# adammoss/nnest

Measured on AMD Instinct MI355X. Metric: live-point evals/sec (flow-transform + loglike) + log-Z error, x_dim=50, higher is better.
Workload: dtype f32

## Files before the change

### nnest_amd/csrc/nnest_solo.hip

```cpp
#include <string.h>
#include <mutex>
#include "mh_common.h"
#include "nnest_internal.h"
#include "solo_loglike.h"
#include "solo_tile.h"

namespace nnest {

#ifdef NNEST_STAMP
#define PSTAMP(v) do { __builtin_amdgcn_sched_barrier(0); v = __builtin_amdgcn_s_memtime(); __builtin_amdgcn_s_waitcnt(0xC07F); __builtin_amdgcn_sched_barrier(0); } while (0)
#define PSTAMP_DRAINED(v) do { __builtin_amdgcn_sched_barrier(0); __builtin_amdgcn_s_waitcnt(0x0070); v = __builtin_amdgcn_s_memtime(); __builtin_amdgcn_s_waitcnt(0xC07F); __builtin_amdgcn_sched_barrier(0); } while (0)
#ifndef NNEST_STAMP_STEPS
#undef STAMP
#define STAMP(v) do { } while (0)
#endif
#else
#define PSTAMP(v) do { } while (0)
#define PSTAMP_DRAINED(v) do { } while (0)
#endif

static constexpr int SOLO_ETAB = 1024;
__device__ double solo_etab_dev[SOLO_ETAB];
__global__ void solo_etab_kernel() {
    const int k = blockIdx.x * blockDim.x + threadIdx.x;
    if (k < SOLO_ETAB) solo_etab_dev[k] = exp(1.0 / (double)(1 + k));
}
hipError_t solo_prepare_device(int device, hipStream_t st) {
    static std::mutex mu;
    static bool done[64];
    std::lock_guard<std::mutex> g(mu);
    if (device < 0 || device >= 64) return hipErrorInvalidDevice;
    if (done[device]) return hipSuccess;
    hipLaunchKernelGGL(solo_etab_kernel, dim3(SOLO_ETAB / 256), dim3(256), 0, st);
    hipError_t e = hipGetLastError();
    if (e == hipSuccess) e = hipStreamSynchronize(st);
    done[device] = e == hipSuccess;
    return e;
}

template <int U>
__global__ void __launch_bounds__(192) solo_image_kernel(const float *__restrict__ packed, float *__restrict__ limg, int D, int net_params) {
    const int lane = threadIdx.x & 63, b = threadIdx.x >> 6;
    SoloNet<U> nb;
    solo_gather<U>(nb, packed + (size_t)(b * 2 + (lane >= 32 ? 1 : 0)) * net_params, D, (b + 1) & 1, b & 1, lane);
    solo4_store<U>(limg, b, nb, lane);
}
hipError_t launch_solo_image(const float *packed, float *limg, const FlowShape &s, hipStream_t st) {
    if (!s.has_solo_image()) return hipErrorInvalidConfiguration;
    switch (s.NT) {
        case 1: hipLaunchKernelGGL(solo_image_kernel<1>, dim3(1), dim3(192), 0, st, packed, limg, s.D, s.net_params); break;
        case 2: hipLaunchKernelGGL(solo_image_kernel<2>, dim3(1), dim3(192), 0, st, packed, limg, s.D, s.net_params); break;
        case 3: hipLaunchKernelGGL(solo_image_kernel<3>, dim3(1), dim3(192), 0, st, packed, limg, s.D, s.net_params); break;
        case 4: hipLaunchKernelGGL(solo_image_kernel<4>, dim3(1), dim3(192), 0, st, packed, limg, s.D, s.net_params); break;
    }
    return hipGetLastError();
}

template <int U, int WPG> constexpr bool solo_lds_weights() { return U >= 3 || WPG > 4; }
template <int U, int WPG> constexpr int solo_reg_blocks() { return !solo_lds_weights<U, WPG>() ? 3 : (WPG == 4 ? 1 : (U <= 2 && WPG == 8 ? 1 : 0)); }

enum { MH_SOLO_LAG_INTERNAL = 8 };
template <int U, bool DBG, int LK, int WPG>
__global__ void __launch_bounds__(64 * (WPG + 2)) mh_kernel_solo(MhArgs a) {
    extern __shared__ __attribute__((aligned(16))) float wlds[];
    __shared__ __attribute__((aligned(16))) float nbuf[2][WPG][16][2 * U];
    __shared__ float ubuf[2][WPG];
    __shared__ __attribute__((aligned(16))) uint32_t rawbuf[4 * WPG * 8 * U];
    __shared__ int acc_lds[2][WPG];
    __shared__ float fsbuf[2];
    __shared__ float fs_exact;
    __shared__ float fs_cand[2];
    __shared__ int vote_sel;
    __shared__ double etab[SOLO_ETAB];
    __shared__ __attribute__((aligned(16))) float x0buf[WPG][16][2 * U];

    const int lane = threadIdx.x & 63, wave = __builtin_amdgcn_readfirstlane(threadIdx.x >> 6);
    const int tile = blockIdx.x;
    const int D = a.s.D, S = a.steps, C = a.C;
    const bool recorded = DBG && a.noise_dz;
    const bool dynamic = (a.flags & NNEST_MH_DYNAMIC_BATCH) != 0;
    const bool use_tab = S + 2 <= SOLO_ETAB;
    const bool exact_all = dynamic && mh_flag_lag(a.flags) == 0;
    const bool direct_votes = (a.flags & NNEST_MH_WINDOW_VOTES_ONLY) == 0;
    const int lag = exact_all ? MH_SOLO_LAG_INTERNAL : mh_flag_lag(a.flags);
    const int warm = dynamic ? min(exact_all ? S : mh_flag_warm(a.flags), S - 1) : 0;
    constexpr bool LDSW = solo_lds_weights<U, WPG>();
    constexpr int RB = solo_reg_blocks<U, WPG>();
    const int ntiles = (C + WPG - 1) / WPG;
    if (tile >= ntiles) {
        if (dynamic && wave == 0) mh_sync_publisher(a.sync, S, exact_all ? S : max(S - lag, warm), ntiles, C, lane, a.sync_err);
        else if (dynamic && (a.flags & (NNEST_MH_SYNC_ZERO_NEXT | NNEST_MH_SYNC_ZERO_PREV))) {
            const size_t W = (size_t)mh_sync_words(S) + 1;
            unsigned long long *other = (a.flags & NNEST_MH_SYNC_ZERO_NEXT) ? a.sync + W : a.sync - W;
            const int nthr = (int)blockDim.x - 64;
            for (size_t i = threadIdx.x - 64; i < W; i += nthr) other[i] = 0ull;
        }
        return;
    }
    unsigned long long p0 = 0, p1 = 0, p2 = 0, p3 = 0, p4 = 0, p5 = 0, p6 = 0, p7 = 0, p8 = 0;
    (void)p0; (void)p1; (void)p2; (void)p3; (void)p4; (void)p5; (void)p6; (void)p7; (void)p8;
    PSTAMP(p0);
    const float *limg = a.img + a.s.solo_image_offset();
    const int j = wave;
    const int pos = lane & 15;
    const bool translate_half = lane >= 32;
    const bool writer_lane = lane < 16;
    const int row = tile * WPG + j;
    const bool ok = row < C;
    SoloNet<U> net[RB > 0 ? RB : 1];
    float z[2][U];
    double logl = 0.0;
    if (wave < WPG) {
        if constexpr (LDSW) {
            if constexpr (RB == 1) solo_image_load<U>(net[0], limg + (size_t)1 * SOLO4_NF * 64, lane);
        } else {
#pragma unroll
            for (int b = 0; b < 3; ++b) solo_image_load<U>(net[b], limg + (size_t)b * SOLO4_NF * 64, lane);
        }
#pragma unroll
        for (int u = 0; u < U; ++u)
#pragma unroll
            for (int c = 0; c < 2; ++c) {
                const int d = 2 * U * pos + 2 * u + c;
                z[c][u] = (ok && d < D) ? a.z[(size_t)row * D + d] : 0.f;
            }
        logl = ok ? a.logl[row] : 0.0;
    }
    if constexpr (LDSW) solo_image_to_lds<64 * (WPG + 2)>(wlds, limg);
    PSTAMP(p1);
    if (dynamic && use_tab)
        for (int k = threadIdx.x; k < S + 2; k += blockDim.x) etab[k] = solo_etab_dev[k];
    PSTAMP(p2);
    __syncthreads();
    PSTAMP(p3);

    if (wave == WPG) {
        const int g = lane & 3, j = min(lane >> 2, WPG - 1);
        const bool gen = lane < 4 * WPG;
        Xoshiro128 rn = xoshiro_seed(a.seed, a.walker_offset + (uint64_t)(tile * WPG + j), (uint32_t)g, NOISE_STREAM_DZ);
        Xoshiro128 ru = xoshiro_seed(a.seed, a.walker_offset + (uint64_t)(tile * WPG + j), 0xffffffffu, NOISE_STREAM_U);
        constexpr int NQ = 8 * WPG * U;
        unsigned long long n0 = 0, n1 = 0, n2 = 0, n_gen = 0, n_all = 0;
        (void)n0; (void)n1; (void)n2; (void)n_gen; (void)n_all;
        auto draw = [&](int k) {
            if (k > S) return;
            STAMP(n0);
            if (!recorded) {
                if (gen) {
#pragma unroll
                    for (int t = 0; t < 2 * U; ++t) {
                        u32x4 r;
                        r.x = xoshiro_next(rn); r.y = xoshiro_next(rn); r.z = xoshiro_next(rn); r.w = xoshiro_next(rn);
                        *reinterpret_cast<u32x4 *>(&rawbuf[lane * 8 * U + 4 * t]) = r;
                    }
                    const float u = xoshiro_uniform(ru);
                    if (g == 0) ubuf[k & 1][j] = u;
                }
                float *nb = &nbuf[k & 1][0][0][0];
#pragma unroll
                for (int i = 0; i < (NQ + 63) / 64; ++i) {
                    const int q = lane + 64 * i;
                    if (NQ % 64 == 0 || q < NQ) {
                        const u32x4 r = *reinterpret_cast<const u32x4 *>(&rawbuf[4 * q]);
                        const int sl = q / (2 * U), qq = q % (2 * U);
                        const int d0 = 32 * (qq >> 1) + 8 * (sl & 3) + 4 * (qq & 1);
                        float o0, o1, o2, o3;
                        box_muller(r.x, r.y, o0, o1);
                        box_muller(r.z, r.w, o2, o3);
                        const f32x4 o = {d0 < D ? o0 : 0.f, d0 + 1 < D ? o1 : 0.f, d0 + 2 < D ? o2 : 0.f, d0 + 3 < D ? o3 : 0.f};
                        *reinterpret_cast<f32x4 *>(nb + (sl >> 2) * 32 * U + d0) = o;
                    }
                }
            }
            if (!dynamic && lane == 0) fsbuf[k & 1] = a.step_size;
            STAMP(n1);
#ifdef NNEST_STAMP
            n_gen += n1 - n0;
#endif
        };
        STAMP(n2);
        draw(0);
        PSTAMP(p4);
        solo_barrier();
        PSTAMP(p5);
        if (S >= 1) {
            draw(1);
            solo_barrier();
            draw(2);
            for (int k = 1; k <= warm; ++k) {
                solo_barrier();
                solo_barrier();
                draw(k + 2);
                solo_barrier();
            }
            for (int k = warm > 0 ? warm + 2 : 2; k <= S; ++k) {
                solo_barrier();
                draw(k + 1);
            }
        }
#ifdef NNEST_STAMP
        { unsigned long long n3 = 0; STAMP(n3); n_all = n3 - n2; }
#endif
#ifdef NNEST_STAMP
        PSTAMP(p8);
        if (a.scale_out && lane == 0 && tile == 0) {
            float *o = a.scale_out;
            o[4] = (float)n_gen; o[5] = (float)n_all;
            o[32] = (float)(p1 - p0); o[33] = (float)(p2 - p1); o[34] = (float)(p3 - p2); o[35] = (float)(p4 - p3); o[36] = (float)(p5 - p4);
            o[37] = (float)(p8 - p5); o[38] = (float)(p8 - p0);
        }
#endif
#ifndef NNEST_STAMP
        if (!dynamic && a.scale_out && lane == 0) {
            const int g0 = (tile * WPG + 15) >> 4;
            if (16 * g0 < (tile + 1) * WPG && 16 * g0 < C) a.scale_out[g0] = a.step_size;
        }
#endif
        return;
    }
    if (wave == WPG + 1) {
        if (!dynamic) return;
        double scale = (double)a.step_size;
        int accept = 0, reject = 0;
        const int last = S - lag;
        const unsigned long long *wbase = a.sync + 2 * mh_sync_counter_words(S) + (size_t)(tile & (MH_SYNC_SHARDS - 1)) * MH_SYNC_STRIDE;
#define SOLO_RELAY_ITERATION(k_, q_)                                                                                        \
        {                                                                                                                   \
            const int k = (k_), want = k - lag;                                                                             \
              \
              \
              \
              \
              \
            asm volatile("s_waitcnt vmcnt(2)" : "+v"(q_) : : "memory");                                                     \
            if (want > warm) {                                                                                              \
                const bool up = mh_window_vote(a.sync, S, want, tile, q_, a.sync_err);                                      \
                if (up) accept += 1; else reject += 1;                                                                      \
                if (accept > reject) scale *= use_tab ? etab[accept] : exp(1.0 / (1 + accept));                             \
                if (accept < reject) scale /= use_tab ? etab[reject] : exp(1.0 / (1 + reject));                             \
            }                                                                                                               \
                   \
             \
            if (lane == 0) {                                                                                                \
                const int *ac = acc_lds[k & 1];                                                                             \
                const bool mine = k - 2 > warm;                                 \
                int acs = 0;                                                                                                \
                _Pragma("unroll") for (int w_ = 0; w_ < WPG; ++w_) acs += ac[w_];                                           \
                mh_sync_post(a.sync, mine ? k - 2 : 0, tile, mine ? acs : 0);                                               \
            }                                                                                                               \
            const int ask = min(max(want + 2, 1), max(last, 1));         \
            const unsigned long long *wp = wbase + (size_t)((ask - 1) >> 5) * MH_SYNC_SHARDS * MH_SYNC_STRIDE;              \
            asm volatile("global_load_dwordx2 %0, %1, off sc1" : "=v"(q_) : "v"(wp) : "memory");                            \
              \
            if (lane == 0) fsbuf[k & 1] = (float)scale;                                                                     \
            solo_barrier();                                                                           \
        }
        unsigned long long qa = 0, qb = 0;
        int k0 = 0;
        if (warm > 0) {
            auto E = [&](int n) { return use_tab ? etab[n] : exp(1.0 / (1 + n)); };
            auto next_scale = [&](int acc, int rej, double sc) {
                if (acc > rej) sc *= E(acc);
                if (acc < rej) sc /= E(rej);
                return sc;
            };
            if (lane == 0) {
                fsbuf[0] = (float)scale;
                fs_cand[0] = (float)next_scale(accept + 1, reject, scale);
                fs_cand[1] = (float)next_scale(accept, reject + 1, scale);
            }
            solo_barrier();
            if (lane == 0) fsbuf[1] = (float)scale;
            solo_barrier();
            for (int k = 1; k <= warm; ++k) {
                solo_barrier();
                if (lane == 0) {
                    const int *ac = acc_lds[k & 1];
                    int acs = 0;
#pragma unroll
                    for (int w_ = 0; w_ < WPG; ++w_) acs += ac[w_];
                    mh_sync_post(a.sync, k, tile, acs);
                    fsbuf[(k + 1) & 1] = (float)scale;
                }
                solo_barrier();
                const bool up = direct_votes ? 2 * mh_sync_total(a.sync, k, ntiles, 0ull, a.sync_err) > C
                                             : mh_window_vote(a.sync, S, k, tile, 0ull, a.sync_err);
                if (up) accept += 1; else reject += 1;
                scale = next_scale(accept, reject, scale);
                if (lane == 0) {
                    vote_sel = up ? 0 : 1;
                    fs_exact = (float)scale;
                    fs_cand[0] = (float)next_scale(accept + 1, reject, scale);
                    fs_cand[1] = (float)next_scale(accept, reject + 1, scale);
                }
                solo_barrier();
            }
            k0 = warm + 2;
        }
        for (int k2 = k0; k2 <= S; k2 += 2) {
            SOLO_RELAY_ITERATION(k2, qa)
            if (k2 + 1 <= S) SOLO_RELAY_ITERATION(k2 + 1, qb)
        }
#undef SOLO_RELAY_ITERATION
        asm volatile("s_waitcnt vmcnt(0)" : "+v"(qa), "+v"(qb) : : "memory");
        if (exact_all) {
            solo_barrier();
            if (lane == 0) {
                const int *ac = acc_lds[S & 1];
                int acs = 0;
#pragma unroll
                for (int w_ = 0; w_ < WPG; ++w_) acs += ac[w_];
                mh_sync_post(a.sync, S, tile, acs);
            }
            const bool up = direct_votes ? 2 * mh_sync_total(a.sync, S, ntiles, 0ull, a.sync_err) > C : mh_window_vote(a.sync, S, S, tile, 0ull, a.sync_err);
            if (up) accept += 1; else reject += 1;
            if (accept > reject) scale *= use_tab ? etab[accept] : exp(1.0 / (1 + accept));
            if (accept < reject) scale /= use_tab ? etab[reject] : exp(1.0 / (1 + reject));
        }
#ifndef NNEST_STAMP
        if (a.scale_out && lane == 0) {
            const int g0 = (tile * WPG + 15) >> 4;
            if (16 * g0 < (tile + 1) * WPG && 16 * g0 < C) a.scale_out[g0] = (float)scale;
        }
#endif
        return;
    }

    const LikeSpec like = a.like;
    const double loglstar = a.loglstar;
    const bool free_mode = (a.flags & NNEST_MH_UNCONSTRAINED) != 0;
    PSTAMP(p4);
    const unsigned sel = translate_half ? 0xffffffffu : 0u;
    const bool h1 = (lane & 16) != 0;
    auto inverse = [&](float (&xs)[2][U]) {
        if constexpr (LDSW) {
            float ld = solo_coupling_inverse4<U>(Solo4Lds{wlds + (size_t)2 * SOLO4_NF * 64, lane}, sel, h1, xs[1], xs[0]);
            if constexpr (RB == 1) ld += solo_coupling_inverse4<U>(Solo4Reg<U>{net[0]}, sel, h1, xs[0], xs[1]);
            else ld += solo_coupling_inverse4<U>(Solo4Lds{wlds + (size_t)1 * SOLO4_NF * 64, lane}, sel, h1, xs[0], xs[1]);
            ld += solo_coupling_inverse4<U>(Solo4Lds{wlds, lane}, sel, h1, xs[1], xs[0]);
            return ld;
        } else {
            float ld;
            solo_coupling_inverse<U, true>(net[2], sel, h1, xs[1], xs[0], ld);
            solo_coupling_inverse<U, false>(net[1], sel, h1, xs[0], xs[1], ld);
            solo_coupling_inverse<U, false>(net[0], sel, h1, xs[1], xs[0], ld);
            return ld;
        }
    };

    float x[2][U];
#pragma unroll
    for (int u = 0; u < U; ++u)
#pragma unroll
        for (int c = 0; c < 2; ++c) x[c][u] = z[c][u];
    float ld = solo_logdet_total(inverse(x));
    int n_acc = 0, n_call = 0;

    auto store_row = [&](float *base, size_t r, const float (&v)[2][U]) {
#pragma unroll
        for (int u = 0; u < U; ++u)
#pragma unroll
            for (int c = 0; c < 2; ++c) {
                const int d = 2 * U * pos + 2 * u + c;
                if (d < D) base[r * D + d] = v[c][u];
            }
    };
    if (writer_lane && a.x) {
#pragma unroll
        for (int u = 0; u < U; ++u)
#pragma unroll
            for (int c = 0; c < 2; ++c) x0buf[j][pos][2 * u + c] = x[c][u];
    }
    if (DBG && writer_lane && ok) {
        if (a.hist_x) store_row(a.hist_x, (size_t)row * (S + 1), x);
        if (a.hist_logl && pos == 0) a.hist_logl[(size_t)row * (S + 1)] = logl;
    }

    float nz[2 * U], u_next = 0.f, fs_next = a.step_size;
    int kbuf = 0;
    auto fetch_noise = [&]() {
        solo_barrier();
        if (!recorded) {
#pragma unroll
            for (int k = 0; k < 2 * U; ++k) nz[k] = nbuf[kbuf & 1][j][pos][k];
            u_next = ubuf[kbuf & 1][j];
        }
        fs_next = fsbuf[kbuf & 1];
        ++kbuf;
    };
    PSTAMP(p5);
    fetch_noise();
    PSTAMP(p6);

    unsigned long long st0 = 0, st1 = 0, st2 = 0, st3 = 0, a_prop = 0, a_inv = 0, a_post = 0, a_tot = 0;
    (void)st0; (void)st1; (void)st2; (void)st3; (void)a_prop; (void)a_inv; (void)a_post; (void)a_tot;
    struct Prop { float zp[2][U], xp[2][U]; float ldp; double lp; bool pre, acc; };
    auto propose = [&](int it, float fs, float (&zp)[2][U], float &u) {
        if (recorded) {
#pragma unroll
            for (int uu = 0; uu < U; ++uu)
#pragma unroll
                for (int c = 0; c < 2; ++c) {
                    const int d = 2 * U * pos + 2 * uu + c;
                    const float dz = (ok && d < D) ? a.noise_dz[((size_t)(it - 1) * C + row) * D + d] : 0.f;
                    zp[c][uu] = __builtin_fmaf(dz, fs, z[c][uu]);
                }
            u = ok ? a.noise_u[(size_t)(it - 1) * C + row] : 1.f;
        } else {
#pragma unroll
            for (int uu = 0; uu < U; ++uu) {
                zp[0][uu] = __builtin_fmaf(nz[2 * uu], fs, z[0][uu]);
                zp[1][uu] = __builtin_fmaf(nz[2 * uu + 1], fs, z[1][uu]);
            }
            u = u_next;
        }
    };
    auto finish = [&](Prop &r, float u) {
#pragma unroll
        for (int c = 0; c < 2; ++c)
#pragma unroll
            for (int uu = 0; uu < U; ++uu) r.xp[c][uu] = r.zp[c][uu];
        STAMP(st1);
        constexpr bool RIDE = LK == NNEST_LIKE_ROSENBROCK;
        r.ldp = RIDE ? inverse(r.xp) : solo_logdet_total(inverse(r.xp));
        STAMP(st2);
        if constexpr (RIDE) r.lp = solo_loglike<U, LK>(like, D, lane, r.xp, &r.ldp);
        int okl = 1;
#pragma unroll
        for (int c = 0; c < 2; ++c)
#pragma unroll
            for (int uu = 0; uu < U; ++uu) okl &= !(r.xp[c][uu] < -1.f || r.xp[c][uu] > 1.f);
        const bool inb = __ballot(okl != 0) == ~0ull;
        float log_ratio = inb ? (r.ldp - ld) : -INFINITY;
        float ratio = fminf(__expf(log_ratio), 1.0f);
        if (log_ratio != log_ratio) ratio = log_ratio;
        r.pre = ok && (u < ratio);
        if constexpr (!RIDE) r.lp = solo_loglike<U, LK>(like, D, lane, r.xp);
        r.acc = r.pre && (r.lp > loglstar);
        if (free_mode) {
            const double lr = inb ? (double)(r.ldp - ld) + (r.lp - logl) : -INFINITY;
            const double rt = fmin(exp(lr), 1.0);
            r.acc = ok && ((double)u < rt);
        }
    };
    auto apply = [&](int it, const Prop &r) {
        n_call += (free_mode ? ok : r.pre) ? 1 : 0;
        n_acc += r.acc ? 1 : 0;
#pragma unroll
        for (int c = 0; c < 2; ++c)
#pragma unroll
            for (int uu = 0; uu < U; ++uu) {
                z[c][uu] = r.acc ? r.zp[c][uu] : z[c][uu];
                x[c][uu] = r.acc ? r.xp[c][uu] : x[c][uu];
            }
        ld = r.acc ? r.ldp : ld;
        logl = r.acc ? r.lp : logl;
        if (dynamic && lane == 0) acc_lds[it & 1][j] = r.acc ? 1 : 0;
        if (DBG && writer_lane && ok) {
            if (a.hist_x) store_row(a.hist_x, (size_t)row * (S + 1) + it, x);
            if (a.hist_logl && pos == 0) a.hist_logl[(size_t)row * (S + 1) + it] = logl;
        }
    };
    Prop cur;
    bool have = false;
    for (int it = 1; it <= S; ++it) {
        STAMP(st0);
        if (!have) {
            float u;
            propose(it, fs_next, cur.zp, u);
            fetch_noise();
            finish(cur, u);
        }
        apply(it, cur);
        have = false;
        if (it <= warm) {
            solo_barrier();
            const float f0 = fs_cand[0], f1 = fs_cand[1];
            Prop c1;
            float u;
            propose(it + 1, f0, cur.zp, u);
            propose(it + 1, f1, c1.zp, u);
            fetch_noise();
            finish(cur, u);
            finish(c1, u);
            solo_barrier();
            if (vote_sel != 0) cur = c1;
            have = true;
            fs_next = fs_exact;
        }
        STAMP(st3);
#ifdef NNEST_STAMP
        a_prop += st1 - st0; a_inv += st2 - st1; a_post += st3 - st2; a_tot += st3 - st0;
#endif
    }
    if (exact_all) solo_barrier();
    PSTAMP(p7);
#ifdef NNEST_STAMP
    if (a.scale_out && lane == 0 && tile == 0) {
        float *o = a.scale_out;
        if (j == 0) { o[0] = (float)a_tot; o[1] = (float)a_prop; o[2] = (float)a_inv; o[3] = (float)a_post; }
        if (j < 4) { o[8 + 2 * j] = (float)a_inv; o[9 + 2 * j] = (float)a_post; }
    }
#endif
    bool all_moved = n_acc > 0;
    if (a.x) {
        bool mine = true;
        if (writer_lane) {
#pragma unroll
            for (int u = 0; u < U; ++u)
#pragma unroll
                for (int c = 0; c < 2; ++c) {
                    const int d = 2 * U * pos + 2 * u + c;
                    const float x0 = x0buf[j][pos][2 * u + c];
                    mine = mine && (d >= D || x[c][u] != x0);
                }
        }
        all_moved = (__ballot(mine) & 0xffffull) == 0xffffull;
    }
    if (writer_lane && ok) {
        store_row(a.z, (size_t)row, z);
        if (a.x) store_row(a.x, (size_t)row, x);
        if (pos == 0) {
            a.logl[row] = logl;
            if (a.n_accept) a.n_accept[row] = n_acc | (all_moved ? NNEST_MH_ALL_MOVED : 0);
            if (a.n_call) a.n_call[row] = n_call;
        }
    }
#ifdef NNEST_STAMP
    PSTAMP_DRAINED(p8);
    if (a.scale_out && lane == 0 && tile == 0 && j == 0) {
        float *o = a.scale_out;
        o[16] = (float)(p1 - p0); o[17] = (float)(p2 - p1); o[18] = (float)(p3 - p2); o[19] = (float)(p4 - p3); o[20] = (float)(p5 - p4);
        o[21] = (float)(p6 - p5); o[22] = (float)(p7 - p6); o[23] = (float)(p8 - p7); o[24] = (float)(p8 - p0);
    }
#endif
}

template <int U>
static __device__ __forceinline__ void slice_normals(uint64_t seed, uint64_t walker, uint32_t step, int pos, int D, float (&e)[2][U]) {
    const int d0 = 2 * U * pos;
    f32x4 q[(2 * U + 3) / 4 + 1];
    const int q0 = d0 >> 2;
#pragma unroll
    for (int k = 0; k < (2 * U + 3) / 4 + 1; ++k) q[k] = noise_normal4(seed, walker, step, (uint32_t)(q0 + k), NOISE_STREAM_DZ);
#pragma unroll
    for (int u = 0; u < U; ++u)
#pragma unroll
        for (int c = 0; c < 2; ++c) {
            const int d = d0 + 2 * u + c, k = (d >> 2) - q0, r = d & 3;
            float v = 0.f;
#pragma unroll
            for (int kk = 0; kk < (2 * U + 3) / 4 + 1; ++kk)
                if (kk == k) v = r == 0 ? q[kk].x : (r == 1 ? q[kk].y : (r == 2 ? q[kk].z : q[kk].w));
            e[c][u] = d < D ? v : 0.f;
        }
}

template <int U, int LK>
__global__ void __launch_bounds__(256) slice_kernel_solo(SliceArgs a, FlowShape s, const float *limg) {
    extern __shared__ __attribute__((aligned(16))) float wlds[];
    __shared__ __attribute__((aligned(16))) float x0buf[4][16][2 * U];
    const int lane = threadIdx.x & 63, wave = __builtin_amdgcn_readfirstlane(threadIdx.x >> 6);
    const int D = s.D, S = a.steps, C = a.C;
    constexpr bool LDSW = solo_lds_weights<U, 4>();
    if constexpr (LDSW) {
        solo_image_to_lds<256>(wlds, limg);
        __syncthreads();
    }
    const int pos = lane & 15;
    const bool translate_half = lane >= 32, writer_lane = lane < 16;
    const int row = blockIdx.x * 4 + wave;
    const bool ok = row < C;
    if (!ok) return;
    const LikeSpec like = a.like;
    const double loglstar = a.loglstar;
    SoloNet<U> net[LDSW ? 1 : 3];
    if constexpr (!LDSW) {
#pragma unroll
        for (int b = 0; b < 3; ++b) solo_image_load<U>(net[b], limg + (size_t)b * SOLO4_NF * 64, lane);
    }
    const unsigned sel = translate_half ? 0xffffffffu : 0u;
    const bool h1 = (lane & 16) != 0;
    auto inverse = [&](float (&xs)[2][U]) {
        if constexpr (LDSW) {
            float ld = solo_coupling_inverse4<U>(Solo4Lds{wlds + (size_t)2 * SOLO4_NF * 64, lane}, sel, h1, xs[1], xs[0]);
            ld += solo_coupling_inverse4<U>(Solo4Lds{wlds + (size_t)1 * SOLO4_NF * 64, lane}, sel, h1, xs[0], xs[1]);
            ld += solo_coupling_inverse4<U>(Solo4Lds{wlds, lane}, sel, h1, xs[1], xs[0]);
            return ld;
        } else {
            float ld;
            solo_coupling_inverse<U, true>(net[2], sel, h1, xs[1], xs[0], ld);
            solo_coupling_inverse<U, false>(net[1], sel, h1, xs[0], xs[1], ld);
            solo_coupling_inverse<U, false>(net[0], sel, h1, xs[1], xs[0], ld);
            return ld;
        }
    };
    auto store_row = [&](float *base, size_t r, const float (&v)[2][U]) {
#pragma unroll
        for (int u = 0; u < U; ++u)
#pragma unroll
            for (int c = 0; c < 2; ++c) {
                const int d = 2 * U * pos + 2 * u + c;
                if (d < D) base[r * D + d] = v[c][u];
            }
    };
    float z[2][U], x[2][U];
#pragma unroll
    for (int u = 0; u < U; ++u)
#pragma unroll
        for (int c = 0; c < 2; ++c) {
            const int d = 2 * U * pos + 2 * u + c;
            z[c][u] = d < D ? a.z[(size_t)row * D + d] : 0.f;
            x[c][u] = z[c][u];
        }
    float ld = solo_logdet_total(inverse(x));
    double logl = a.logl[row];
    if (writer_lane && a.x) {
#pragma unroll
        for (int u = 0; u < U; ++u)
#pragma unroll
            for (int c = 0; c < 2; ++c) x0buf[wave][pos][2 * u + c] = x[c][u];
    }
    if (writer_lane && a.hist_x) store_row(a.hist_x, (size_t)row * (S + 1), x);
    const uint64_t walker = a.walker_offset + (uint64_t)row;
    int n_call = 0, n_move = 0, n_eval = 0;
    float zc[2][U], xc[2][U], ldc = 0.f;
    double lc = 0.0;
    for (int it = 1; it <= S; ++it) {
        float e[2][U];
        if (a.noise_dz) {
#pragma unroll
            for (int u = 0; u < U; ++u)
#pragma unroll
                for (int c = 0; c < 2; ++c) {
                    const int d = 2 * U * pos + 2 * u + c;
                    e[c][u] = d < D ? a.noise_dz[((size_t)(it - 1) * C + row) * D + d] : 0.f;
                }
        } else {
            slice_normals<U>(a.seed, walker, (uint32_t)it, pos, D, e);
        }
        const float u0 = noise_uniform(a.seed, walker, 64u * (uint32_t)it + 0u), u1 = noise_uniform(a.seed, walker, 64u * (uint32_t)it + 1u);
        const float logy = ld + __logf(u1);
        auto inside = [&](float t) -> bool {
            const float tw = t * a.width;
#pragma unroll
            for (int u = 0; u < U; ++u)
#pragma unroll
                for (int c = 0; c < 2; ++c) { zc[c][u] = __builtin_fmaf(e[c][u], tw, z[c][u]); xc[c][u] = zc[c][u]; }
            ldc = solo_logdet_total(inverse(xc));
            int okl = 1;
#pragma unroll
            for (int c = 0; c < 2; ++c)
#pragma unroll
                for (int u = 0; u < U; ++u) okl &= !(xc[c][u] < -1.f || xc[c][u] > 1.f);
            const bool inb = __ballot(okl != 0) == ~0ull;
            const bool pre = inb && (ldc > logy);
            lc = solo_loglike<U, LK>(like, D, lane, xc);
            n_eval += 1;
            n_call += pre ? 1 : 0;
            return pre && (lc > loglstar);
        };
        float tl = -u0, tr = 1.0f - u0;
        if (a.max_out > 0) {
            const int B = 2 * a.max_out;
            int n = 0;
            while (n <= B && inside(tl)) { tl -= 1.0f; n += 1; }
            while (n <= B && inside(tr)) { tr += 1.0f; n += 1; }
            if (n > B) {
                tl = -u0;
                tr = 1.0f - u0;
                const int nl = slice_stepout_left(a.seed, walker, (uint32_t)it, a.max_out);
                for (int j = 0; j < nl; ++j) { if (!inside(tl)) break; tl -= 1.0f; }
                for (int j = 0; j < B - nl; ++j) { if (!inside(tr)) break; tr += 1.0f; }
            }
        }
        bool moved = false;
        for (int k = 0; k < a.max_shrink; ++k) {
            const float uk = noise_uniform(a.seed, walker, 64u * (uint32_t)it + 2u + (uint32_t)k);
            const float t = __builtin_fmaf(tr - tl, uk, tl);
            if (inside(t)) { moved = true; break; }
            if (t < 0.f) tl = t; else tr = t;
        }
        if (moved) {
#pragma unroll
            for (int c = 0; c < 2; ++c)
#pragma unroll
                for (int u = 0; u < U; ++u) { z[c][u] = zc[c][u]; x[c][u] = xc[c][u]; }
            ld = ldc; logl = lc; n_move += 1;
        }
        if (writer_lane && a.hist_x) store_row(a.hist_x, (size_t)row * (S + 1) + it, x);
    }
    bool all_moved = n_move > 0;
    if (a.x) {
        bool mine = true;
        if (writer_lane) {
#pragma unroll
            for (int u = 0; u < U; ++u)
#pragma unroll
                for (int c = 0; c < 2; ++c) {
                    const int d = 2 * U * pos + 2 * u + c;
                    const float x0 = x0buf[wave][pos][2 * u + c];
                    mine = mine && (d >= D || x[c][u] != x0);
                }
        }
        all_moved = (__ballot(mine) & 0xffffull) == 0xffffull;
    }
    if (writer_lane) {
        store_row(a.z, (size_t)row, z);
        if (a.x) store_row(a.x, (size_t)row, x);
        if (pos == 0) {
            a.logl[row] = logl;
            if (a.n_call) a.n_call[row] = n_call;
            if (a.n_move) a.n_move[row] = n_move | (all_moved ? NNEST_MH_ALL_MOVED : 0);
            if (a.n_eval) a.n_eval[row] = n_eval;
        }
    }
}

__global__ void slice_fill_noise_kernel(float *__restrict__ dz, int steps, int C, int D, uint64_t seed, uint64_t walker_offset) {
    const long nq = (long)steps * C * ((D + 3) / 4);
    for (long i = (long)blockIdx.x * blockDim.x + threadIdx.x; i < nq; i += (long)gridDim.x * blockDim.x) {
        const int Q = (D + 3) / 4, q = (int)(i % Q), c = (int)((i / Q) % C), it = (int)(i / ((long)Q * C)) + 1;
        const f32x4 n = noise_normal4(seed, walker_offset + (uint64_t)c, (uint32_t)it, (uint32_t)q, NOISE_STREAM_DZ);
        float *o = dz + ((size_t)(it - 1) * C + c) * D + 4 * q;
        if (4 * q + 0 < D) o[0] = n.x;
        if (4 * q + 1 < D) o[1] = n.y;
        if (4 * q + 2 < D) o[2] = n.z;
        if (4 * q + 3 < D) o[3] = n.w;
    }
}

template <int U, int LK>
static hipError_t launch_slice_k(const FlowShape &s, const float *limg, const SliceArgs &a, hipStream_t st) {
    const size_t lds = solo_lds_weights<U, 4>() ? (size_t)3 * SOLO4_NF * 64 * sizeof(float) : 0;
    hipError_t e = hipFuncSetAttribute(reinterpret_cast<const void *>(slice_kernel_solo<U, LK>), hipFuncAttributeMaxDynamicSharedMemorySize, (int)lds);
    if (e != hipSuccess) return e;
    hipLaunchKernelGGL((slice_kernel_solo<U, LK>), dim3((a.C + 3) / 4), dim3(256), lds, st, a, s, limg);
    return hipGetLastError();
}

bool slice_form_eligible(const FlowShape &s) {
    return s.kind == FLOW_KIND_NVP && s.H == 16 && s.B == 3 && s.L == 1 && s.scale_mode == 0 && s.NT >= 1 && s.NT <= 4;
}

hipError_t launch_slice_solo(const FlowShape &s, const float *limg, const SliceArgs &a, hipStream_t st) {
    if (a.C <= 0) return hipSuccess;
    if (!slice_form_eligible(s)) return hipErrorInvalidConfiguration;
    const bool rosen = a.like.id == NNEST_LIKE_ROSENBROCK;
    switch (s.NT) {
        case 1: return rosen ? launch_slice_k<1, NNEST_LIKE_ROSENBROCK>(s, limg, a, st) : launch_slice_k<1, -1>(s, limg, a, st);
        case 2: return rosen ? launch_slice_k<2, NNEST_LIKE_ROSENBROCK>(s, limg, a, st) : launch_slice_k<2, -1>(s, limg, a, st);
        case 3: return rosen ? launch_slice_k<3, NNEST_LIKE_ROSENBROCK>(s, limg, a, st) : launch_slice_k<3, -1>(s, limg, a, st);
        case 4: return rosen ? launch_slice_k<4, NNEST_LIKE_ROSENBROCK>(s, limg, a, st) : launch_slice_k<4, -1>(s, limg, a, st);
    }
    return hipErrorInvalidConfiguration;
}

hipError_t launch_slice_fill_noise(float *dz, int steps, int C, int D, uint64_t seed, uint64_t walker_offset, hipStream_t st) {
    hipLaunchKernelGGL(slice_fill_noise_kernel, dim3(256), dim3(256), 0, st, dz, steps, C, D, seed, walker_offset);
    return hipGetLastError();
}

int solo_walkers_per_group(int C, int num_cu) {
    static const int pinned = [] { const char *e = getenv("NNEST_SOLO_WPG"); return e ? atoi(e) : 0; }();
    for (int wpg = 4; wpg <= 12; wpg += 4) {
        if (pinned && wpg != pinned) continue;
        if ((C + wpg - 1) / wpg + 1 <= num_cu) return wpg;
    }
    return 0;
}

bool solo_form_eligible(const MhArgs &a, int num_cu) {
    const FlowShape &s = a.s;
    if (s.H != 16 || s.B != 3 || s.L != 1 || s.scale_mode != 0 || s.NT < 1 || s.NT > 4) return false;
    if (a.flags & NNEST_MH_DYNAMIC_STEP) return false;
    if ((a.flags & NNEST_MH_DYNAMIC_BATCH) && (mh_flag_lag(a.flags) == 1 || mh_flag_lag(a.flags) == 2)) return false;
    const int wpg = solo_walkers_per_group(a.C, num_cu);
    if (wpg != 4 && (a.noise_dz || a.hist_x || a.hist_logl)) return false;
    return wpg != 0;
}

template <int U, bool DBG, int LK, int WPG>
static hipError_t launch_solo_k(const MhArgs &a, hipStream_t st) {
    const int batch = (a.flags & NNEST_MH_DYNAMIC_BATCH) ? 1 : 0;
    const int grid = (a.C + WPG - 1) / WPG + batch;
    const size_t lds = solo_lds_weights<U, WPG>() ? (size_t)3 * SOLO4_NF * 64 * sizeof(float) : 0;
    hipError_t e = hipFuncSetAttribute(reinterpret_cast<const void *>(mh_kernel_solo<U, DBG, LK, WPG>),
                                       hipFuncAttributeMaxDynamicSharedMemorySize, (int)lds);
    if (e != hipSuccess) return e;
    hipLaunchKernelGGL((mh_kernel_solo<U, DBG, LK, WPG>), dim3(grid), dim3(64 * (WPG + 2)), lds, st, a);
    return hipGetLastError();
}
template <int U, bool DBG, int LK>
static hipError_t launch_solo_w(const MhArgs &a, int wpg, hipStream_t st) {
    if (wpg == 4) return launch_solo_k<U, DBG, LK, 4>(a, st);
    if constexpr (!DBG) {
        if (wpg == 8) return launch_solo_k<U, DBG, LK, 8>(a, st);
        if (wpg == 12) return launch_solo_k<U, DBG, LK, 12>(a, st);
    }
    return hipErrorInvalidConfiguration;
}

hipError_t launch_mh_solo(const MhArgs &a_in, int num_cu, hipStream_t st) {
    MhArgs a = a_in;
    static const bool window_votes = [] { const char *e = getenv("NNEST_SOLO_VOTE"); return e && !strcmp(e, "window"); }();
    if (window_votes) a.flags |= NNEST_MH_WINDOW_VOTES_ONLY;
    const bool dbg = a.noise_dz || a.hist_x || a.hist_logl;
    const int wpg = solo_walkers_per_group(a.C, num_cu);
    if (!dbg && a.like.id == NNEST_LIKE_ROSENBROCK) {
        if (a.s.NT == 1) return launch_solo_w<1, false, NNEST_LIKE_ROSENBROCK>(a, wpg, st);
        if (a.s.NT == 2) return launch_solo_w<2, false, NNEST_LIKE_ROSENBROCK>(a, wpg, st);
        if (a.s.NT == 3) return launch_solo_w<3, false, NNEST_LIKE_ROSENBROCK>(a, wpg, st);
        if (a.s.NT == 4) return launch_solo_w<4, false, NNEST_LIKE_ROSENBROCK>(a, wpg, st);
    }
    switch (a.s.NT) {
        case 1: return dbg ? launch_solo_w<1, true, -1>(a, wpg, st) : launch_solo_w<1, false, -1>(a, wpg, st);
        case 2: return dbg ? launch_solo_w<2, true, -1>(a, wpg, st) : launch_solo_w<2, false, -1>(a, wpg, st);
        case 3: return dbg ? launch_solo_w<3, true, -1>(a, wpg, st) : launch_solo_w<3, false, -1>(a, wpg, st);
        case 4: return dbg ? launch_solo_w<4, true, -1>(a, wpg, st) : launch_solo_w<4, false, -1>(a, wpg, st);
    }
    return hipErrorInvalidConfiguration;
}

}
```

Before: 941.8 million.

## Restructure solo MH loop into warm and unrolled straight phases, defer x inverse

Splits the MH step loop into a warm-up phase and a straight phase unrolled by two, so the LDS double-buffer parity is a compile-time constant instead of a running counter. Proposal registers are pinned across the noise-fetch barrier to steer scheduling. When neither DBG nor LDS weights are in use, x is no longer selected at every step; it is rebuilt once at the end by running the inverse flow on z. The intent is to cut per-step register moves and selects, at the cost of one extra flow inverse per chain and extra code size.

```diff
diff --git a/nnest_amd/csrc/nnest_solo.hip b/nnest_amd/csrc/nnest_solo.hip
--- a/nnest_amd/csrc/nnest_solo.hip
+++ b/nnest_amd/csrc/nnest_solo.hip
@@ -3,6 +3,7 @@
 #include "mh_common.h"
 #include "nnest_internal.h"
 #include "solo_loglike.h"
+#include "solo_schedule.h"
 #include "solo_tile.h"
 
 namespace nnest {
@@ -58,6 +59,14 @@
 
 template <int U, int WPG> constexpr bool solo_lds_weights() { return U >= 3 || WPG > 4; }
 template <int U, int WPG> constexpr int solo_reg_blocks() { return !solo_lds_weights<U, WPG>() ? 3 : (WPG == 4 ? 1 : (U <= 2 && WPG == 8 ? 1 : 0)); }
+
+template <int U>
+static __device__ __forceinline__ void solo_pin(float (&v)[2][U]) {
+#pragma unroll
+    for (int c = 0; c < 2; ++c)
+#pragma unroll
+        for (int u = 0; u < U; ++u) asm volatile("" : "+v"(v[c][u]));
+}
 
 enum { MH_SOLO_LAG_INTERNAL = 8 };
 template <int U, bool DBG, int LK, int WPG>
@@ -83,7 +92,7 @@
     const bool exact_all = dynamic && mh_flag_lag(a.flags) == 0;
     const bool direct_votes = (a.flags & NNEST_MH_WINDOW_VOTES_ONLY) == 0;
     const int lag = exact_all ? MH_SOLO_LAG_INTERNAL : mh_flag_lag(a.flags);
-    const int warm = dynamic ? min(exact_all ? S : mh_flag_warm(a.flags), S - 1) : 0;
+    const int warm = solo_warm_steps(S, mh_flag_warm(a.flags), dynamic, exact_all);
     constexpr bool LDSW = solo_lds_weights<U, WPG>();
     constexpr int RB = solo_reg_blocks<U, WPG>();
     const int ntiles = (C + WPG - 1) / WPG;
@@ -193,7 +202,7 @@
                 draw(k + 2);
                 solo_barrier();
             }
-            for (int k = warm > 0 ? warm + 2 : 2; k <= S; ++k) {
+            for (int k = solo_first_lagged_fetch(warm); k <= S; ++k) {
                 solo_barrier();
                 draw(k + 1);
             }
@@ -256,7 +265,7 @@
             solo_barrier();                                                                           \
         }
         unsigned long long qa = 0, qb = 0;
-        int k0 = 0;
+        const int k0 = solo_relay_first_iteration(warm);
         if (warm > 0) {
             auto E = [&](int n) { return use_tab ? etab[n] : exp(1.0 / (1 + n)); };
             auto next_scale = [&](int acc, int rej, double sc) {
@@ -295,7 +304,6 @@
                 }
                 solo_barrier();
             }
-            k0 = warm + 2;
         }
         for (int k2 = k0; k2 <= S; k2 += 2) {
             SOLO_RELAY_ITERATION(k2, qa)
@@ -348,6 +356,7 @@
         }
     };
 
+    constexpr bool X_LATE = !DBG && !LDSW;
     float x[2][U];
 #pragma unroll
     for (int u = 0; u < U; ++u)
@@ -377,19 +386,18 @@
     }
 
     float nz[2 * U], u_next = 0.f, fs_next = a.step_size;
-    int kbuf = 0;
-    auto fetch_noise = [&]() {
+    auto fetch_noise = [&](int par, auto &...zp) {
         solo_barrier();
+        (solo_pin(zp), ...);
         if (!recorded) {
 #pragma unroll
-            for (int k = 0; k < 2 * U; ++k) nz[k] = nbuf[kbuf & 1][j][pos][k];
-            u_next = ubuf[kbuf & 1][j];
-        }
-        fs_next = fsbuf[kbuf & 1];
-        ++kbuf;
+            for (int k = 0; k < 2 * U; ++k) nz[k] = nbuf[par][j][pos][k];
+            u_next = ubuf[par][j];
+        }
+        fs_next = fsbuf[par];
     };
     PSTAMP(p5);
-    fetch_noise();
+    fetch_noise(0);
     PSTAMP(p6);
 
     unsigned long long st0 = 0, st1 = 0, st2 = 0, st3 = 0, a_prop = 0, a_inv = 0, a_post = 0, a_tot = 0;
@@ -443,7 +451,7 @@
             r.acc = ok && ((double)u < rt);
         }
     };
-    auto apply = [&](int it, const Prop &r) {
+    auto apply = [&](int it, int par, const Prop &r) {
         n_call += (free_mode ? ok : r.pre) ? 1 : 0;
         n_acc += r.acc ? 1 : 0;
 #pragma unroll
@@ -451,47 +459,67 @@
 #pragma unroll
             for (int uu = 0; uu < U; ++uu) {
                 z[c][uu] = r.acc ? r.zp[c][uu] : z[c][uu];
-                x[c][uu] = r.acc ? r.xp[c][uu] : x[c][uu];
+                if constexpr (!X_LATE) x[c][uu] = r.acc ? r.xp[c][uu] : x[c][uu];
             }
         ld = r.acc ? r.ldp : ld;
         logl = r.acc ? r.lp : logl;
-        if (dynamic && lane == 0) acc_lds[it & 1][j] = r.acc ? 1 : 0;
+        if (dynamic && lane == 0) acc_lds[par][j] = r.acc ? 1 : 0;
         if (DBG && writer_lane && ok) {
             if (a.hist_x) store_row(a.hist_x, (size_t)row * (S + 1) + it, x);
             if (a.hist_logl && pos == 0) a.hist_logl[(size_t)row * (S + 1) + it] = logl;
         }
     };
-    Prop cur;
-    bool have = false;
-    for (int it = 1; it <= S; ++it) {
-        STAMP(st0);
-        if (!have) {
+    if (warm > 0) {
+        Prop cur;
+        {
             float u;
-            propose(it, fs_next, cur.zp, u);
-            fetch_noise();
+            propose(1, fs_next, cur.zp, u);
+            fetch_noise(1, cur.zp);
             finish(cur, u);
         }
-        apply(it, cur);
-        have = false;
-        if (it <= warm) {
+        for (int it = 1; it <= warm; ++it) {
+            STAMP(st0);
+            apply(it, it & 1, cur);
             solo_barrier();
             const float f0 = fs_cand[0], f1 = fs_cand[1];
             Prop c1;
             float u;
             propose(it + 1, f0, cur.zp, u);
             propose(it + 1, f1, c1.zp, u);
-            fetch_noise();
+            fetch_noise((it + 1) & 1, cur.zp, c1.zp);
             finish(cur, u);
             finish(c1, u);
             solo_barrier();
             if (vote_sel != 0) cur = c1;
-            have = true;
             fs_next = fs_exact;
-        }
+            STAMP(st3);
+#ifdef NNEST_STAMP
+            a_prop += st1 - st0; a_inv += st2 - st1; a_post += st3 - st2; a_tot += st3 - st0;
+#endif
+        }
+        apply(warm + 1, (warm + 1) & 1, cur);
+    }
+    auto straight_step = [&](int it, int par) {
+        STAMP(st0);
+        Prop r;
+        float u;
+        propose(it, fs_next, r.zp, u);
+        fetch_noise(par, r.zp);
+        finish(r, u);
+        apply(it, par, r);
         STAMP(st3);
 #ifdef NNEST_STAMP
         a_prop += st1 - st0; a_inv += st2 - st1; a_post += st3 - st2; a_tot += st3 - st0;
 #endif
+    };
+    {
+        int it = solo_first_straight_step(warm);
+        if (it <= S && (it & 1)) { straight_step(it, 1); ++it; }
+        for (; it < S; it += 2) {
+            straight_step(it, 0);
+            straight_step(it + 1, 1);
+        }
+        if (it <= S) straight_step(it, 0);
     }
     if (exact_all) solo_barrier();
     PSTAMP(p7);
@@ -504,6 +532,13 @@
 #endif
     bool all_moved = n_acc > 0;
     if (a.x) {
+        if constexpr (X_LATE) {
+#pragma unroll
+            for (int u = 0; u < U; ++u)
+#pragma unroll
+                for (int c = 0; c < 2; ++c) x[c][u] = z[c][u];
+            (void)inverse(x);
+        }
         bool mine = true;
         if (writer_lane) {
 #pragma unroll
diff --git a/nnest_amd/csrc/solo_schedule.h b/nnest_amd/csrc/solo_schedule.h
--- /dev/null
+++ b/nnest_amd/csrc/solo_schedule.h
@@ -0,0 +1,45 @@
+#pragma once
+
+#if defined(__HIPCC__) || defined(__CUDACC__)
+#define SOLO_SCHED_FN __host__ __device__ constexpr
+#else
+#define SOLO_SCHED_FN constexpr
+#endif
+
+namespace nnest {
+
+SOLO_SCHED_FN int solo_warm_steps(int S, int flag_warm, bool dynamic, bool exact_all) {
+    return dynamic ? ((exact_all ? S : flag_warm) < S - 1 ? (exact_all ? S : flag_warm) : S - 1) : 0;
+}
+SOLO_SCHED_FN int solo_first_straight_step(int warm) { return warm > 0 ? warm + 2 : 1; }
+SOLO_SCHED_FN int solo_first_lagged_fetch(int warm) { return warm > 0 ? warm + 2 : 2; }
+SOLO_SCHED_FN int solo_lagged_fetches(int S, int warm) { return S >= solo_first_lagged_fetch(warm) ? S - solo_first_lagged_fetch(warm) + 1 : 0; }
+SOLO_SCHED_FN int solo_relay_first_iteration(int warm) { return warm > 0 ? warm + 2 : 0; }
+
+SOLO_SCHED_FN int solo_net_barriers(int S, int warm, bool dynamic, bool exact_all) {
+    int n = 1;
+    if (warm > 0) n += 1 + 3 * warm;
+    const int first = solo_first_straight_step(warm);
+    n += S >= first ? S - first + 1 : 0;
+    return n + (exact_all ? 1 : 0);
+}
+SOLO_SCHED_FN int solo_noise_barriers(int S, int warm, bool dynamic, bool exact_all) {
+    int n = 1;
+    if (S >= 1) n += 1 + 3 * warm + solo_lagged_fetches(S, warm);
+    return n;
+}
+SOLO_SCHED_FN int solo_relay_barriers(int S, int warm, bool dynamic, bool exact_all) {
+    if (!dynamic) return 0;
+    int n = warm > 0 ? 2 + 3 * warm : 0;
+    const int k0 = solo_relay_first_iteration(warm);
+    n += S >= k0 ? S - k0 + 1 : 0;
+    return n + (exact_all ? 1 : 0);
+}
+SOLO_SCHED_FN int solo_noise_barriers_due(int S, int warm, bool dynamic, bool exact_all) {
+    return solo_net_barriers(S, warm, dynamic, exact_all) - (exact_all ? 1 : 0);
+}
+SOLO_SCHED_FN int solo_relay_barriers_due(int S, int warm, bool dynamic, bool exact_all) {
+    return dynamic ? solo_net_barriers(S, warm, dynamic, exact_all) : 0;
+}
+
+}
diff --git a/profiles/r09/k4_solo_loop.s b/profiles/r09/k4_solo_loop.s
--- /dev/null
+++ b/profiles/r09/k4_solo_loop.s
@@ -0,0 +1,812 @@
+	v_mov_b32_e32 v193, s70
+	ds_write_b32 v193, v185 offset:16
+	s_or_b64 exec, exec, s[12:13]
+	v_and_b32_e32 v186, 0xffff, v186
+	v_and_b32_e32 v147, 0xffff, v147
+	s_add_i32 s19, s19, 2
+	v_add3_u32 v168, v168, v186, v147
+	v_add3_u32 v169, v169, v187, v185
+	v_cndmask_b32_e64 v29, v29, v190, s[14:15]
+	v_cndmask_b32_e64 v93, v93, v191, s[14:15]
+	v_cndmask_b32_e64 v143, v143, v189, s[14:15]
+	v_cndmask_b32_e64 v145, v145, v167, s[14:15]
+	v_cndmask_b32_e64 v144, v144, v166, s[14:15]
+	v_cndmask_b32_e64 v177, v177, v192, s[14:15]
+	s_cmp_lt_i32 s19, s29
+	v_cndmask_b32_e64 v89, v89, v188, s[14:15]
+	s_cbranch_scc0 1220
+	s_waitcnt lgkmcnt(0)
+	v_fma_f32 v189, v138, v171, v29
+	v_fma_f32 v188, v139, v171, v143
+	v_fma_f32 v190, v140, v171, v93
+	v_fma_f32 v171, v141, v171, v89
+	s_waitcnt lgkmcnt(0)
+	s_barrier
+	v_mov_b32_e32 v198, v146
+	v_mov_b32_e32 v147, v188
+	v_mov_b32_e32 v166, v171
+	v_bfi_b32 v187, v173, v190, v189
+	v_mov_b32_dpp v147, v188 row_ror:8 row_mask:0xa bank_mask:0xf
+	v_mov_b32_dpp v166, v171 row_ror:8 row_mask:0xa bank_mask:0xf
+	v_fma_f32 v167, v147, v94, v90
+	v_mul_f32_e32 v186, v166, v102
+	v_fmac_f32_dpp v186, v166, v103 row_ror:1 row_mask:0xf bank_mask:0xf
+	v_fmac_f32_dpp v167, v147, v95 row_ror:1 row_mask:0xf bank_mask:0xf
+	v_fmac_f32_dpp v186, v166, v104 row_ror:2 row_mask:0xf bank_mask:0xf
+	v_fmac_f32_dpp v167, v147, v96 row_ror:2 row_mask:0xf bank_mask:0xf
+	v_fmac_f32_dpp v186, v166, v105 row_ror:3 row_mask:0xf bank_mask:0xf
+	v_fmac_f32_dpp v167, v147, v97 row_ror:3 row_mask:0xf bank_mask:0xf
+	v_fmac_f32_dpp v186, v166, v106 row_ror:4 row_mask:0xf bank_mask:0xf
+	v_fmac_f32_dpp v167, v147, v98 row_ror:4 row_mask:0xf bank_mask:0xf
+	v_fmac_f32_dpp v186, v166, v107 row_ror:5 row_mask:0xf bank_mask:0xf
+	v_fmac_f32_dpp v167, v147, v99 row_ror:5 row_mask:0xf bank_mask:0xf
+	v_fmac_f32_dpp v186, v166, v108 row_ror:6 row_mask:0xf bank_mask:0xf
+	v_fmac_f32_dpp v167, v147, v100 row_ror:6 row_mask:0xf bank_mask:0xf
+	v_fmac_f32_dpp v186, v166, v109 row_ror:7 row_mask:0xf bank_mask:0xf
+	v_fmac_f32_dpp v167, v147, v101 row_ror:7 row_mask:0xf bank_mask:0xf
+	v_add_f32_e32 v166, v167, v186
+	v_mov_b32_dpp v147, v186 row_ror:8 row_mask:0xf bank_mask:0xf
+	v_add_f32_dpp v147, v167, v147 row_ror:8 row_mask:0xf bank_mask:0xf
+	s_nop 1
+	v_permlane16_swap_b32_e32 v166, v147
+	v_add_f32_e32 v167, v166, v147
+	v_exp_f32_e32 v147, v167
+	v_max_f32_e32 v166, 0, v167
+	v_add_f32_e32 v147, 1.0, v147
+	v_rcp_f32_e32 v147, v147
+	s_nop 0
+	v_fma_f32 v147, v147, -2.0, 1.0
+	v_bfi_b32 v167, v142, v166, v147
+	v_fma_f32 v147, v167, v110, v91
+	s_nop 0
+	v_mul_f32_dpp v166, v167, v111 row_ror:1 row_mask:0xf bank_mask:0xf
+	v_fmac_f32_dpp v147, v167, v112 row_ror:2 row_mask:0xf bank_mask:0xf
+	v_fmac_f32_dpp v166, v167, v113 row_ror:3 row_mask:0xf bank_mask:0xf
+	v_fmac_f32_dpp v147, v167, v114 row_ror:4 row_mask:0xf bank_mask:0xf
+	v_fmac_f32_dpp v166, v167, v115 row_ror:5 row_mask:0xf bank_mask:0xf
+	v_fmac_f32_dpp v147, v167, v116 row_ror:6 row_mask:0xf bank_mask:0xf
+	v_fmac_f32_dpp v166, v167, v117 row_ror:7 row_mask:0xf bank_mask:0xf
+	v_add_f32_e32 v167, v147, v166
+	v_add_f32_e32 v186, v147, v166
+	s_nop 1
+	v_permlane16_swap_b32_e32 v167, v186
+	v_add_f32_e32 v167, v167, v186
+	v_exp_f32_e32 v147, v167
+	v_max_f32_e32 v166, 0, v167
+	v_add_f32_e32 v147, 1.0, v147
+	v_rcp_f32_e32 v147, v147
+	s_nop 0
+	v_fma_f32 v147, v147, -2.0, 1.0
+	v_bfi_b32 v167, v142, v166, v147
+	v_fma_f32 v147, v167, v118, v92
+	v_mov_b32_e32 v166, 0
+	v_fmac_f32_dpp v166, v167, v122 row_ror:8 row_mask:0xf bank_mask:0xf
+	v_fmac_f32_dpp v147, v167, v119 row_ror:1 row_mask:0xf bank_mask:0xf
+	v_fmac_f32_dpp v166, v167, v123 row_ror:9 row_mask:0xf bank_mask:0xf
+	v_fmac_f32_dpp v147, v167, v120 row_ror:2 row_mask:0xf bank_mask:0xf
+	v_fmac_f32_dpp v166, v167, v124 row_ror:10 row_mask:0xf bank_mask:0xf
+	v_fmac_f32_dpp v147, v167, v121 row_ror:3 row_mask:0xf bank_mask:0xf
+	v_fmac_f32_dpp v166, v167, v125 row_ror:11 row_mask:0xf bank_mask:0xf
+	v_fmac_f32_dpp v147, v167, v126 row_ror:4 row_mask:0xf bank_mask:0xf
+	v_fmac_f32_dpp v166, v167, v130 row_ror:12 row_mask:0xf bank_mask:0xf
+	v_fmac_f32_dpp v147, v167, v127 row_ror:5 row_mask:0xf bank_mask:0xf
+	v_fmac_f32_dpp v166, v167, v131 row_ror:13 row_mask:0xf bank_mask:0xf
+	v_fmac_f32_dpp v147, v167, v128 row_ror:6 row_mask:0xf bank_mask:0xf
+	v_fmac_f32_dpp v166, v167, v132 row_ror:14 row_mask:0xf bank_mask:0xf
+	v_fmac_f32_dpp v147, v167, v129 row_ror:7 row_mask:0xf bank_mask:0xf
+	v_fmac_f32_dpp v166, v167, v133 row_ror:15 row_mask:0xf bank_mask:0xf
+	v_add_f32_e32 v167, v147, v166
+	v_add_f32_e32 v186, v147, v166
+	s_nop 1
+	v_permlane32_swap_b32_e32 v167, v186
+	v_mul_f32_e32 v147, 0xbfb8aa3b, v167
+	v_exp_f32_e32 v147, v147
+	v_sub_f32_e32 v166, v187, v186
+	v_mul_f32_e32 v193, v166, v147
+	v_mul_f32_e32 v194, v166, v147
+	v_mul_f32_e32 v191, -1.0, v167
+	s_nop 0
+	v_permlane16_swap_b32_e32 v193, v194
+	ds_read_b128 v[138:141], v176
+	ds_read_b32 v185, v178
+	ds_read_b32 v192, v179 offset:12352
+	v_mov_b32_e32 v147, v193
+	v_mov_b32_e32 v167, v194
+	v_bfi_b32 v195, v173, v171, v188
+	v_mov_b32_dpp v147, v193 row_ror:8 row_mask:0xa bank_mask:0xf
+	v_mov_b32_dpp v167, v194 row_ror:8 row_mask:0xa bank_mask:0xf
+	v_fma_f32 v186, v147, v50, v86
+	v_mul_f32_e32 v187, v167, v34
+	v_fmac_f32_dpp v187, v167, v35 row_ror:1 row_mask:0xf bank_mask:0xf
+	v_fmac_f32_dpp v186, v147, v51 row_ror:1 row_mask:0xf bank_mask:0xf
+	v_fmac_f32_dpp v187, v167, v36 row_ror:2 row_mask:0xf bank_mask:0xf
+	v_fmac_f32_dpp v186, v147, v52 row_ror:2 row_mask:0xf bank_mask:0xf
+	v_fmac_f32_dpp v187, v167, v37 row_ror:3 row_mask:0xf bank_mask:0xf
+	v_fmac_f32_dpp v186, v147, v53 row_ror:3 row_mask:0xf bank_mask:0xf
+	v_fmac_f32_dpp v187, v167, v58 row_ror:4 row_mask:0xf bank_mask:0xf
+	v_fmac_f32_dpp v186, v147, v54 row_ror:4 row_mask:0xf bank_mask:0xf
+	v_fmac_f32_dpp v187, v167, v59 row_ror:5 row_mask:0xf bank_mask:0xf
+	v_fmac_f32_dpp v186, v147, v55 row_ror:5 row_mask:0xf bank_mask:0xf
+	v_fmac_f32_dpp v187, v167, v60 row_ror:6 row_mask:0xf bank_mask:0xf
+	v_fmac_f32_dpp v186, v147, v56 row_ror:6 row_mask:0xf bank_mask:0xf
+	v_fmac_f32_dpp v187, v167, v61 row_ror:7 row_mask:0xf bank_mask:0xf
+	v_fmac_f32_dpp v186, v147, v57 row_ror:7 row_mask:0xf bank_mask:0xf
+	v_add_f32_e32 v167, v186, v187
+	v_mov_b32_dpp v147, v187 row_ror:8 row_mask:0xf bank_mask:0xf
+	v_add_f32_dpp v147, v186, v147 row_ror:8 row_mask:0xf bank_mask:0xf
+	s_nop 1
+	v_permlane16_swap_b32_e32 v167, v147
+	v_add_f32_e32 v186, v167, v147
+	v_exp_f32_e32 v147, v186
+	v_max_f32_e32 v167, 0, v186
+	v_add_f32_e32 v147, 1.0, v147
+	v_rcp_f32_e32 v147, v147
+	s_nop 0
+	v_fma_f32 v147, v147, -2.0, 1.0
+	v_bfi_b32 v186, v142, v167, v147
+	v_fma_f32 v147, v186, v62, v87
+	s_nop 0
+	v_mul_f32_dpp v167, v186, v63 row_ror:1 row_mask:0xf bank_mask:0xf
+	v_fmac_f32_dpp v147, v186, v64 row_ror:2 row_mask:0xf bank_mask:0xf
+	v_fmac_f32_dpp v167, v186, v65 row_ror:3 row_mask:0xf bank_mask:0xf
+	v_fmac_f32_dpp v147, v186, v66 row_ror:4 row_mask:0xf bank_mask:0xf
+	v_fmac_f32_dpp v167, v186, v67 row_ror:5 row_mask:0xf bank_mask:0xf
+	v_fmac_f32_dpp v147, v186, v68 row_ror:6 row_mask:0xf bank_mask:0xf
+	v_fmac_f32_dpp v167, v186, v69 row_ror:7 row_mask:0xf bank_mask:0xf
+	v_add_f32_e32 v186, v147, v167
+	v_add_f32_e32 v187, v147, v167
+	s_nop 1
+	v_permlane16_swap_b32_e32 v186, v187
+	v_add_f32_e32 v186, v186, v187
+	v_exp_f32_e32 v147, v186
+	v_max_f32_e32 v167, 0, v186
+	v_add_f32_e32 v147, 1.0, v147
+	v_rcp_f32_e32 v147, v147
+	s_nop 0
+	v_fma_f32 v147, v147, -2.0, 1.0
+	v_bfi_b32 v186, v142, v167, v147
+	v_fma_f32 v147, v186, v70, v88
+	v_mov_b32_e32 v167, 0
+	v_fmac_f32_dpp v167, v186, v78 row_ror:8 row_mask:0xf bank_mask:0xf
+	v_fmac_f32_dpp v147, v186, v71 row_ror:1 row_mask:0xf bank_mask:0xf
+	v_fmac_f32_dpp v167, v186, v79 row_ror:9 row_mask:0xf bank_mask:0xf
+	v_fmac_f32_dpp v147, v186, v72 row_ror:2 row_mask:0xf bank_mask:0xf
+	v_fmac_f32_dpp v167, v186, v80 row_ror:10 row_mask:0xf bank_mask:0xf
+	v_fmac_f32_dpp v147, v186, v73 row_ror:3 row_mask:0xf bank_mask:0xf
+	v_fmac_f32_dpp v167, v186, v81 row_ror:11 row_mask:0xf bank_mask:0xf
+	v_fmac_f32_dpp v147, v186, v74 row_ror:4 row_mask:0xf bank_mask:0xf
+	v_fmac_f32_dpp v167, v186, v82 row_ror:12 row_mask:0xf bank_mask:0xf
+	v_fmac_f32_dpp v147, v186, v75 row_ror:5 row_mask:0xf bank_mask:0xf
+	v_fmac_f32_dpp v167, v186, v83 row_ror:13 row_mask:0xf bank_mask:0xf
+	v_fmac_f32_dpp v147, v186, v76 row_ror:6 row_mask:0xf bank_mask:0xf
+	v_fmac_f32_dpp v167, v186, v84 row_ror:14 row_mask:0xf bank_mask:0xf
+	v_fmac_f32_dpp v147, v186, v77 row_ror:7 row_mask:0xf bank_mask:0xf
+	v_fmac_f32_dpp v167, v186, v85 row_ror:15 row_mask:0xf bank_mask:0xf
+	v_add_f32_e32 v186, v147, v167
+	v_add_f32_e32 v187, v147, v167
+	s_nop 1
+	v_permlane32_swap_b32_e32 v186, v187
+	v_mul_f32_e32 v147, 0xbfb8aa3b, v186
+	v_exp_f32_e32 v147, v147
+	v_sub_f32_e32 v167, v195, v187
+	v_mul_f32_e32 v166, v167, v147
+	v_mul_f32_e32 v202, v167, v147
+	v_sub_f32_e32 v191, v191, v186
+	s_nop 0
+	v_permlane16_swap_b32_e32 v166, v202
+	s_nop 0
+	v_mov_b32_e32 v147, v166
+	v_mov_b32_e32 v187, v202
+	v_bfi_b32 v197, v173, v194, v193
+	v_mov_b32_dpp v147, v166 row_ror:8 row_mask:0xa bank_mask:0xf
+	v_mov_b32_dpp v187, v202 row_ror:8 row_mask:0xa bank_mask:0xf
+	v_fma_f32 v195, v147, v30, v26
+	v_mul_f32_e32 v196, v187, v42
+	v_fmac_f32_dpp v196, v187, v43 row_ror:1 row_mask:0xf bank_mask:0xf
+	v_fmac_f32_dpp v195, v147, v31 row_ror:1 row_mask:0xf bank_mask:0xf
+	v_fmac_f32_dpp v196, v187, v44 row_ror:2 row_mask:0xf bank_mask:0xf
+	v_fmac_f32_dpp v195, v147, v32 row_ror:2 row_mask:0xf bank_mask:0xf
+	v_fmac_f32_dpp v196, v187, v45 row_ror:3 row_mask:0xf bank_mask:0xf
+	v_fmac_f32_dpp v195, v147, v33 row_ror:3 row_mask:0xf bank_mask:0xf
+	v_fmac_f32_dpp v196, v187, v46 row_ror:4 row_mask:0xf bank_mask:0xf
+	v_fmac_f32_dpp v195, v147, v38 row_ror:4 row_mask:0xf bank_mask:0xf
+	v_fmac_f32_dpp v196, v187, v47 row_ror:5 row_mask:0xf bank_mask:0xf
+	v_fmac_f32_dpp v195, v147, v39 row_ror:5 row_mask:0xf bank_mask:0xf
+	v_fmac_f32_dpp v196, v187, v48 row_ror:6 row_mask:0xf bank_mask:0xf
+	v_fmac_f32_dpp v195, v147, v40 row_ror:6 row_mask:0xf bank_mask:0xf
+	v_fmac_f32_dpp v196, v187, v49 row_ror:7 row_mask:0xf bank_mask:0xf
+	v_fmac_f32_dpp v195, v147, v41 row_ror:7 row_mask:0xf bank_mask:0xf
+	v_add_f32_e32 v187, v195, v196
+	v_mov_b32_dpp v147, v196 row_ror:8 row_mask:0xf bank_mask:0xf
+	v_add_f32_dpp v147, v195, v147 row_ror:8 row_mask:0xf bank_mask:0xf
+	s_nop 1
+	v_permlane16_swap_b32_e32 v187, v147
+	v_add_f32_e32 v195, v187, v147
+	v_exp_f32_e32 v147, v195
+	v_max_f32_e32 v187, 0, v195
+	v_add_f32_e32 v147, 1.0, v147
+	v_rcp_f32_e32 v147, v147
+	s_nop 0
+	v_fma_f32 v147, v147, -2.0, 1.0
+	v_bfi_b32 v195, v142, v187, v147
+	v_fma_f32 v147, v195, v6, v27
+	s_nop 0
+	v_mul_f32_dpp v187, v195, v7 row_ror:1 row_mask:0xf bank_mask:0xf
+	v_fmac_f32_dpp v147, v195, v8 row_ror:2 row_mask:0xf bank_mask:0xf
+	v_fmac_f32_dpp v187, v195, v9 row_ror:3 row_mask:0xf bank_mask:0xf
+	v_fmac_f32_dpp v147, v195, v14 row_ror:4 row_mask:0xf bank_mask:0xf
+	v_fmac_f32_dpp v187, v195, v15 row_ror:5 row_mask:0xf bank_mask:0xf
+	v_fmac_f32_dpp v147, v195, v16 row_ror:6 row_mask:0xf bank_mask:0xf
+	v_fmac_f32_dpp v187, v195, v17 row_ror:7 row_mask:0xf bank_mask:0xf
+	v_add_f32_e32 v195, v147, v187
+	v_add_f32_e32 v196, v147, v187
+	s_nop 1
+	v_permlane16_swap_b32_e32 v195, v196
+	v_add_f32_e32 v195, v195, v196
+	v_exp_f32_e32 v147, v195
+	v_max_f32_e32 v187, 0, v195
+	v_add_f32_e32 v147, 1.0, v147
+	v_rcp_f32_e32 v147, v147
+	s_nop 0
+	v_fma_f32 v147, v147, -2.0, 1.0
+	v_bfi_b32 v195, v142, v187, v147
+	v_fma_f32 v147, v195, v2, v28
+	v_mov_b32_e32 v187, 0
+	v_fmac_f32_dpp v187, v195, v18 row_ror:8 row_mask:0xf bank_mask:0xf
+	v_fmac_f32_dpp v147, v195, v3 row_ror:1 row_mask:0xf bank_mask:0xf
+	v_fmac_f32_dpp v187, v195, v19 row_ror:9 row_mask:0xf bank_mask:0xf
+	v_fmac_f32_dpp v147, v195, v4 row_ror:2 row_mask:0xf bank_mask:0xf
+	v_fmac_f32_dpp v187, v195, v20 row_ror:10 row_mask:0xf bank_mask:0xf
+	v_fmac_f32_dpp v147, v195, v5 row_ror:3 row_mask:0xf bank_mask:0xf
+	v_fmac_f32_dpp v187, v195, v21 row_ror:11 row_mask:0xf bank_mask:0xf
+	v_fmac_f32_dpp v147, v195, v10 row_ror:4 row_mask:0xf bank_mask:0xf
+	v_fmac_f32_dpp v187, v195, v22 row_ror:12 row_mask:0xf bank_mask:0xf
+	v_fmac_f32_dpp v147, v195, v11 row_ror:5 row_mask:0xf bank_mask:0xf
+	v_fmac_f32_dpp v187, v195, v23 row_ror:13 row_mask:0xf bank_mask:0xf
+	v_fmac_f32_dpp v147, v195, v12 row_ror:6 row_mask:0xf bank_mask:0xf
+	v_fmac_f32_dpp v187, v195, v24 row_ror:14 row_mask:0xf bank_mask:0xf
+	v_fmac_f32_dpp v147, v195, v13 row_ror:7 row_mask:0xf bank_mask:0xf
+	v_fmac_f32_dpp v187, v195, v25 row_ror:15 row_mask:0xf bank_mask:0xf
+	v_add_f32_e32 v195, v147, v187
+	v_add_f32_e32 v196, v147, v187
+	s_nop 1
+	v_permlane32_swap_b32_e32 v195, v196
+	v_mul_f32_e32 v147, 0xbfb8aa3b, v195
+	v_exp_f32_e32 v147, v147
+	v_sub_f32_e32 v187, v197, v196
+	v_mul_f32_e32 v167, v187, v147
+	v_mul_f32_e32 v186, v187, v147
+	v_sub_f32_e32 v191, v191, v195
+	s_nop 0
+	v_permlane16_swap_b32_e32 v167, v186
+	s_nop 0
+	v_pk_mul_f32 v[194:195], s[52:53], v[166:167]
+	v_mov_b32_e32 v187, v166
+	v_pk_mul_f32 v[196:197], s[52:53], v[186:187]
+	v_pk_mul_f32 v[200:201], v[194:195], v[194:195] neg_lo:[0,1] neg_hi:[0,1]
+	v_mov_b32_dpp v199, v195 row_ror:15 row_mask:0xf bank_mask:0xf bound_ctrl:1
+	v_pk_add_f32 v[200:201], v[196:197], v[200:201]
+	v_pk_add_f32 v[194:195], v[194:195], 1.0 op_sel_hi:[1,0] neg_lo:[1,0] neg_hi:[1,0]
+	v_pk_mul_f32 v[200:201], v[200:201], v[200:201]
+	v_pk_mul_f32 v[194:195], v[194:195], v[194:195]
+	v_pk_mul_f32 v[200:201], v[200:201], s[18:19] op_sel_hi:[1,0]
+	s_nop 0
+	v_pk_add_f32 v[194:195], v[194:195], v[200:201]
+	s_nop 0
+	v_cndmask_b32_e64 v147, 0, v195, s[2:3]
+	v_cndmask_b32_e64 v187, 0, v194, s[4:5]
+	v_pk_mul_f32 v[194:195], v[196:197], v[196:197]
+	v_add_f32_e32 v187, v187, v147
+	v_mul_f32_e32 v147, s52, v202
+	v_mov_b32_e32 v197, v194
+	v_pk_add_f32 v[194:195], v[146:147], v[196:197] neg_lo:[0,1] neg_hi:[0,1]
+	s_nop 0
+	v_pk_mul_f32 v[194:195], v[194:195], v[194:195]
+	s_nop 0
+	v_mul_f32_e32 v193, 0x42c80000, v195
+	v_add_f32_e32 v193, v194, v193
+	v_mul_f32_e32 v195, v147, v147
+	v_mov_b32_e32 v194, v147
+	v_pk_add_f32 v[194:195], v[198:199], v[194:195] neg_lo:[0,1] neg_hi:[0,1]
+	v_cndmask_b32_e64 v193, 0, v193, s[6:7]
+	v_pk_mul_f32 v[194:195], v[194:195], v[194:195]
+	v_add_f32_e32 v187, v193, v187
+	v_mul_f32_e32 v147, 0x42c80000, v195
+	v_add_f32_e32 v147, v194, v147
+	v_cndmask_b32_e64 v147, 0, v147, s[8:9]
+	v_add_f32_e32 v147, v147, v187
+	s_nop 1
+	v_add_f32_dpp v191, v191, v191 row_ror:8 row_mask:0xf bank_mask:0xf bound_ctrl:1
+	v_add_f32_dpp v147, v147, v147 row_ror:8 row_mask:0xf bank_mask:0xf bound_ctrl:1
+	s_nop 0
+	v_add_f32_dpp v191, v191, v191 row_ror:4 row_mask:0xf bank_mask:0xf bound_ctrl:1
+	v_add_f32_dpp v147, v147, v147 row_ror:4 row_mask:0xf bank_mask:0xf bound_ctrl:1
+	s_nop 0
+	v_add_f32_dpp v191, v191, v191 row_ror:2 row_mask:0xf bank_mask:0xf bound_ctrl:1
+	v_add_f32_dpp v147, v147, v147 row_ror:2 row_mask:0xf bank_mask:0xf bound_ctrl:1
+	s_nop 0
+	v_add_f32_dpp v187, v191, v191 row_ror:1 row_mask:0xf bank_mask:0xf bound_ctrl:1
+	v_add_f32_dpp v191, v191, v191 row_ror:1 row_mask:0xf bank_mask:0xf bound_ctrl:1
+	v_add_f32_dpp v147, v147, v147 row_ror:1 row_mask:0xf bank_mask:0xf bound_ctrl:1
+	s_nop 0
+	v_permlane16_swap_b32_e32 v191, v187
+	v_add_f32_e32 v191, v191, v187
+	s_nop 0
+	v_cvt_f64_f32_e32 v[194:195], v147
+	v_max3_f32 v147, |v202|, |v166|, |v186|
+	v_max_f32_e64 v166, |v167|, |v167|
+	v_max_f32_e32 v147, v147, v166
+	v_cmp_nlt_f32_e32 vcc, 1.0, v147
+	s_cmp_eq_u64 vcc, -1
+	v_sub_f32_e32 v147, v191, v177
+	s_cselect_b64 s[12:13], -1, 0
+	v_cndmask_b32_e64 v186, v182, v147, s[12:13]
+	v_mul_f32_e32 v166, 0x3fb8aa3b, v186
+	v_exp_f32_e32 v187, v166
+	v_cmp_le_f64_e64 vcc, |v[194:195]|, s[54:55]
+	v_min_f32_e32 v187, 1.0, v187
+	s_nop 0
+	v_cndmask_b32_e64 v167, v180, -v195, vcc
+	v_cndmask_b32_e32 v166, v181, v194, vcc
+	v_cmp_u_f32_e32 vcc, v186, v186
+	v_cmp_lt_f64_e64 s[14:15], s[26:27], v[166:167]
+	s_nop 0
+	v_cndmask_b32_e32 v186, v187, v186, vcc
+	v_cmp_lt_f32_e32 vcc, v170, v186
+	s_and_b64 s[68:69], s[50:51], vcc
+	s_and_b64 vcc, exec, s[10:11]
+	s_and_b64 s[14:15], s[68:69], s[14:15]
+	s_cbranch_vccnz 62
+	v_cvt_f64_f32_e32 v[186:187], v147
+	v_add_f64 v[194:195], v[166:167], -v[144:145]
+	v_add_f64 v[186:187], v[194:195], v[186:187]
+	v_cndmask_b32_e64 v187, v183, v187, s[12:13]
+	v_cndmask_b32_e64 v186, 0, v186, s[12:13]
+	v_mul_f64 v[194:195], v[186:187], s[56:57]
+	v_rndne_f64_e32 v[194:195], v[194:195]
+	v_fma_f64 v[196:197], s[58:59], v[194:195], v[186:187]
+	v_fmac_f64_e32 v[196:197], s[60:61], v[194:195]
+	v_mov_b64_e32 v[198:199], v[148:149]
+	v_fmac_f64_e32 v[198:199], s[62:63], v[196:197]
+	v_mov_b64_e32 v[200:201], v[150:151]
+	v_fmac_f64_e32 v[200:201], v[196:197], v[198:199]
+	v_mov_b64_e32 v[198:199], v[152:153]
+	v_fmac_f64_e32 v[198:199], v[196:197], v[200:201]
+	v_mov_b64_e32 v[200:201], v[154:155]
+	v_fmac_f64_e32 v[200:201], v[196:197], v[198:199]
+	v_mov_b64_e32 v[198:199], v[156:157]
+	v_fmac_f64_e32 v[198:199], v[196:197], v[200:201]
+	v_mov_b64_e32 v[200:201], v[158:159]
+	v_fmac_f64_e32 v[200:201], v[196:197], v[198:199]
+	v_mov_b64_e32 v[198:199], v[160:161]
+	v_fmac_f64_e32 v[198:199], v[196:197], v[200:201]
+	v_mov_b64_e32 v[200:201], v[162:163]
+	v_fmac_f64_e32 v[200:201], v[196:197], v[198:199]
+	v_mov_b64_e32 v[198:199], v[164:165]
+	v_fmac_f64_e32 v[198:199], v[196:197], v[200:201]
+	v_fma_f64 v[198:199], v[196:197], v[198:199], 1.0
+	v_fma_f64 v[196:197], v[196:197], v[198:199], 1.0
+	v_cvt_i32_f64_e32 v147, v[194:195]
+	v_ldexp_f64 v[194:195], v[196:197], v147
+	v_min_f64 v[194:195], v[194:195], 1.0
+	v_cmp_nlt_f64_e32 vcc, s[64:65], v[186:187]
+	v_cmp_ngt_f64_e64 s[12:13], s[66:67], v[186:187]
+	s_andn2_b64 s[14:15], s[14:15], exec
+	v_cndmask_b32_e32 v147, v184, v195, vcc
+	s_and_b64 vcc, s[12:13], vcc
+	v_cndmask_b32_e64 v187, 0, v147, s[12:13]
+	v_cndmask_b32_e32 v186, 0, v194, vcc
+	v_cvt_f64_f32_e32 v[194:195], v170
+	v_cmp_gt_f64_e32 vcc, v[186:187], v[194:195]
+	s_and_b64 s[12:13], s[50:51], vcc
+	s_and_b64 s[12:13], s[12:13], exec
+	s_or_b64 s[14:15], s[14:15], s[12:13]
+	v_mov_b32_e32 v186, v175
+	v_cndmask_b32_e64 v187, 0, 1, s[14:15]
+	s_and_saveexec_b64 s[12:13], s[16:17]
+	s_cbranch_execnz 6
+	s_branch 8
+	v_cndmask_b32_e64 v186, 0, 1, s[68:69]
+	v_cndmask_b32_e64 v187, 0, 1, s[14:15]
+	s_and_saveexec_b64 s[12:13], s[16:17]
+	v_mov_b32_e32 v147, s70
+	ds_write_b32 v147, v187
+	s_or_b64 exec, exec, s[12:13]
+	v_cndmask_b32_e64 v29, v29, v189, s[14:15]
+	v_cndmask_b32_e64 v93, v93, v190, s[14:15]
+	v_cndmask_b32_e64 v143, v143, v188, s[14:15]
+	v_cndmask_b32_e64 v89, v89, v171, s[14:15]
+	v_cndmask_b32_e64 v177, v177, v191, s[14:15]
+	s_waitcnt lgkmcnt(0)
+	v_fma_f32 v190, v138, v192, v29
+	v_fma_f32 v189, v139, v192, v143
+	v_fma_f32 v191, v140, v192, v93
+	v_fma_f32 v188, v141, v192, v89
+	v_mov_b32_e32 v147, s81
+	v_cndmask_b32_e64 v145, v145, v167, s[14:15]
+	v_cndmask_b32_e64 v144, v144, v166, s[14:15]
+	s_waitcnt lgkmcnt(0)
+	s_barrier
+	ds_read_b128 v[138:141], v176 offset:1024
+	ds_read_b32 v170, v147 offset:16
+	ds_read_b32 v171, v179 offset:12356
+	v_mov_b32_e32 v147, v189
+	v_mov_b32_e32 v166, v188
+	v_bfi_b32 v194, v173, v191, v190
+	v_mov_b32_dpp v147, v189 row_ror:8 row_mask:0xa bank_mask:0xf
+	v_mov_b32_dpp v166, v188 row_ror:8 row_mask:0xa bank_mask:0xf
+	v_fma_f32 v167, v147, v94, v90
+	v_mul_f32_e32 v193, v166, v102
+	v_fmac_f32_dpp v193, v166, v103 row_ror:1 row_mask:0xf bank_mask:0xf
+	v_fmac_f32_dpp v167, v147, v95 row_ror:1 row_mask:0xf bank_mask:0xf
+	v_fmac_f32_dpp v193, v166, v104 row_ror:2 row_mask:0xf bank_mask:0xf
+	v_fmac_f32_dpp v167, v147, v96 row_ror:2 row_mask:0xf bank_mask:0xf
+	v_fmac_f32_dpp v193, v166, v105 row_ror:3 row_mask:0xf bank_mask:0xf
+	v_fmac_f32_dpp v167, v147, v97 row_ror:3 row_mask:0xf bank_mask:0xf
+	v_fmac_f32_dpp v193, v166, v106 row_ror:4 row_mask:0xf bank_mask:0xf
+	v_fmac_f32_dpp v167, v147, v98 row_ror:4 row_mask:0xf bank_mask:0xf
+	v_fmac_f32_dpp v193, v166, v107 row_ror:5 row_mask:0xf bank_mask:0xf
+	v_fmac_f32_dpp v167, v147, v99 row_ror:5 row_mask:0xf bank_mask:0xf
+	v_fmac_f32_dpp v193, v166, v108 row_ror:6 row_mask:0xf bank_mask:0xf
+	v_fmac_f32_dpp v167, v147, v100 row_ror:6 row_mask:0xf bank_mask:0xf
+	v_fmac_f32_dpp v193, v166, v109 row_ror:7 row_mask:0xf bank_mask:0xf
+	v_fmac_f32_dpp v167, v147, v101 row_ror:7 row_mask:0xf bank_mask:0xf
+	v_add_f32_e32 v166, v167, v193
+	v_mov_b32_dpp v147, v193 row_ror:8 row_mask:0xf bank_mask:0xf
+	v_add_f32_dpp v147, v167, v147 row_ror:8 row_mask:0xf bank_mask:0xf
+	s_nop 1
+	v_permlane16_swap_b32_e32 v166, v147
+	v_add_f32_e32 v167, v166, v147
+	v_exp_f32_e32 v147, v167
+	v_max_f32_e32 v166, 0, v167
+	v_add_f32_e32 v147, 1.0, v147
+	v_rcp_f32_e32 v147, v147
+	s_nop 0
+	v_fma_f32 v147, v147, -2.0, 1.0
+	v_bfi_b32 v167, v142, v166, v147
+	v_fma_f32 v147, v167, v110, v91
+	s_nop 0
+	v_mul_f32_dpp v166, v167, v111 row_ror:1 row_mask:0xf bank_mask:0xf
+	v_fmac_f32_dpp v147, v167, v112 row_ror:2 row_mask:0xf bank_mask:0xf
+	v_fmac_f32_dpp v166, v167, v113 row_ror:3 row_mask:0xf bank_mask:0xf
+	v_fmac_f32_dpp v147, v167, v114 row_ror:4 row_mask:0xf bank_mask:0xf
+	v_fmac_f32_dpp v166, v167, v115 row_ror:5 row_mask:0xf bank_mask:0xf
+	v_fmac_f32_dpp v147, v167, v116 row_ror:6 row_mask:0xf bank_mask:0xf
+	v_fmac_f32_dpp v166, v167, v117 row_ror:7 row_mask:0xf bank_mask:0xf
+	v_add_f32_e32 v167, v147, v166
+	v_add_f32_e32 v193, v147, v166
+	s_nop 1
+	v_permlane16_swap_b32_e32 v167, v193
+	v_add_f32_e32 v167, v167, v193
+	v_exp_f32_e32 v147, v167
+	v_max_f32_e32 v166, 0, v167
+	v_add_f32_e32 v147, 1.0, v147
+	v_rcp_f32_e32 v147, v147
+	s_nop 0
+	v_fma_f32 v147, v147, -2.0, 1.0
+	v_bfi_b32 v167, v142, v166, v147
+	v_fma_f32 v147, v167, v118, v92
+	v_mov_b32_e32 v166, 0
+	v_fmac_f32_dpp v166, v167, v122 row_ror:8 row_mask:0xf bank_mask:0xf
+	v_fmac_f32_dpp v147, v167, v119 row_ror:1 row_mask:0xf bank_mask:0xf
+	v_fmac_f32_dpp v166, v167, v123 row_ror:9 row_mask:0xf bank_mask:0xf
+	v_fmac_f32_dpp v147, v167, v120 row_ror:2 row_mask:0xf bank_mask:0xf
+	v_fmac_f32_dpp v166, v167, v124 row_ror:10 row_mask:0xf bank_mask:0xf
+	v_fmac_f32_dpp v147, v167, v121 row_ror:3 row_mask:0xf bank_mask:0xf
+	v_fmac_f32_dpp v166, v167, v125 row_ror:11 row_mask:0xf bank_mask:0xf
+	v_fmac_f32_dpp v147, v167, v126 row_ror:4 row_mask:0xf bank_mask:0xf
+	v_fmac_f32_dpp v166, v167, v130 row_ror:12 row_mask:0xf bank_mask:0xf
+	v_fmac_f32_dpp v147, v167, v127 row_ror:5 row_mask:0xf bank_mask:0xf
+	v_fmac_f32_dpp v166, v167, v131 row_ror:13 row_mask:0xf bank_mask:0xf
+	v_fmac_f32_dpp v147, v167, v128 row_ror:6 row_mask:0xf bank_mask:0xf
+	v_fmac_f32_dpp v166, v167, v132 row_ror:14 row_mask:0xf bank_mask:0xf
+	v_fmac_f32_dpp v147, v167, v129 row_ror:7 row_mask:0xf bank_mask:0xf
+	v_fmac_f32_dpp v166, v167, v133 row_ror:15 row_mask:0xf bank_mask:0xf
+	v_add_f32_e32 v167, v147, v166
+	v_add_f32_e32 v193, v147, v166
+	s_nop 1
+	v_permlane32_swap_b32_e32 v167, v193
+	v_mul_f32_e32 v147, 0xbfb8aa3b, v167
+	v_exp_f32_e32 v147, v147
+	v_sub_f32_e32 v166, v194, v193
+	v_mul_f32_e32 v195, v166, v147
+	v_mul_f32_e32 v196, v166, v147
+	v_mul_f32_e32 v192, -1.0, v167
+	s_nop 0
+	v_permlane16_swap_b32_e32 v195, v196
+	v_mov_b32_e32 v200, v146
+	v_mov_b32_e32 v147, v195
+	v_mov_b32_e32 v167, v196
+	v_bfi_b32 v197, v173, v188, v189
+	v_mov_b32_dpp v147, v195 row_ror:8 row_mask:0xa bank_mask:0xf
+	v_mov_b32_dpp v167, v196 row_ror:8 row_mask:0xa bank_mask:0xf
+	v_fma_f32 v193, v147, v50, v86
+	v_mul_f32_e32 v194, v167, v34
+	v_fmac_f32_dpp v194, v167, v35 row_ror:1 row_mask:0xf bank_mask:0xf
+	v_fmac_f32_dpp v193, v147, v51 row_ror:1 row_mask:0xf bank_mask:0xf
+	v_fmac_f32_dpp v194, v167, v36 row_ror:2 row_mask:0xf bank_mask:0xf
+	v_fmac_f32_dpp v193, v147, v52 row_ror:2 row_mask:0xf bank_mask:0xf
+	v_fmac_f32_dpp v194, v167, v37 row_ror:3 row_mask:0xf bank_mask:0xf
+	v_fmac_f32_dpp v193, v147, v53 row_ror:3 row_mask:0xf bank_mask:0xf
+	v_fmac_f32_dpp v194, v167, v58 row_ror:4 row_mask:0xf bank_mask:0xf
+	v_fmac_f32_dpp v193, v147, v54 row_ror:4 row_mask:0xf bank_mask:0xf
+	v_fmac_f32_dpp v194, v167, v59 row_ror:5 row_mask:0xf bank_mask:0xf
+	v_fmac_f32_dpp v193, v147, v55 row_ror:5 row_mask:0xf bank_mask:0xf
+	v_fmac_f32_dpp v194, v167, v60 row_ror:6 row_mask:0xf bank_mask:0xf
+	v_fmac_f32_dpp v193, v147, v56 row_ror:6 row_mask:0xf bank_mask:0xf
+	v_fmac_f32_dpp v194, v167, v61 row_ror:7 row_mask:0xf bank_mask:0xf
+	v_fmac_f32_dpp v193, v147, v57 row_ror:7 row_mask:0xf bank_mask:0xf
+	v_add_f32_e32 v167, v193, v194
+	v_mov_b32_dpp v147, v194 row_ror:8 row_mask:0xf bank_mask:0xf
+	v_add_f32_dpp v147, v193, v147 row_ror:8 row_mask:0xf bank_mask:0xf
+	s_nop 1
+	v_permlane16_swap_b32_e32 v167, v147
+	v_add_f32_e32 v193, v167, v147
+	v_exp_f32_e32 v147, v193
+	v_max_f32_e32 v167, 0, v193
+	v_add_f32_e32 v147, 1.0, v147
+	v_rcp_f32_e32 v147, v147
+	s_nop 0
+	v_fma_f32 v147, v147, -2.0, 1.0
+	v_bfi_b32 v193, v142, v167, v147
+	v_fma_f32 v147, v193, v62, v87
+	s_nop 0
+	v_mul_f32_dpp v167, v193, v63 row_ror:1 row_mask:0xf bank_mask:0xf
+	v_fmac_f32_dpp v147, v193, v64 row_ror:2 row_mask:0xf bank_mask:0xf
+	v_fmac_f32_dpp v167, v193, v65 row_ror:3 row_mask:0xf bank_mask:0xf
+	v_fmac_f32_dpp v147, v193, v66 row_ror:4 row_mask:0xf bank_mask:0xf
+	v_fmac_f32_dpp v167, v193, v67 row_ror:5 row_mask:0xf bank_mask:0xf
+	v_fmac_f32_dpp v147, v193, v68 row_ror:6 row_mask:0xf bank_mask:0xf
+	v_fmac_f32_dpp v167, v193, v69 row_ror:7 row_mask:0xf bank_mask:0xf
+	v_add_f32_e32 v193, v147, v167
+	v_add_f32_e32 v194, v147, v167
+	s_nop 1
+	v_permlane16_swap_b32_e32 v193, v194
+	v_add_f32_e32 v193, v193, v194
+	v_exp_f32_e32 v147, v193
+	v_max_f32_e32 v167, 0, v193
+	v_add_f32_e32 v147, 1.0, v147
+	v_rcp_f32_e32 v147, v147
+	s_nop 0
+	v_fma_f32 v147, v147, -2.0, 1.0
+	v_bfi_b32 v193, v142, v167, v147
+	v_fma_f32 v147, v193, v70, v88
+	v_mov_b32_e32 v167, 0
+	v_fmac_f32_dpp v167, v193, v78 row_ror:8 row_mask:0xf bank_mask:0xf
+	v_fmac_f32_dpp v147, v193, v71 row_ror:1 row_mask:0xf bank_mask:0xf
+	v_fmac_f32_dpp v167, v193, v79 row_ror:9 row_mask:0xf bank_mask:0xf
+	v_fmac_f32_dpp v147, v193, v72 row_ror:2 row_mask:0xf bank_mask:0xf
+	v_fmac_f32_dpp v167, v193, v80 row_ror:10 row_mask:0xf bank_mask:0xf
+	v_fmac_f32_dpp v147, v193, v73 row_ror:3 row_mask:0xf bank_mask:0xf
+	v_fmac_f32_dpp v167, v193, v81 row_ror:11 row_mask:0xf bank_mask:0xf
+	v_fmac_f32_dpp v147, v193, v74 row_ror:4 row_mask:0xf bank_mask:0xf
+	v_fmac_f32_dpp v167, v193, v82 row_ror:12 row_mask:0xf bank_mask:0xf
+	v_fmac_f32_dpp v147, v193, v75 row_ror:5 row_mask:0xf bank_mask:0xf
+	v_fmac_f32_dpp v167, v193, v83 row_ror:13 row_mask:0xf bank_mask:0xf
+	v_fmac_f32_dpp v147, v193, v76 row_ror:6 row_mask:0xf bank_mask:0xf
+	v_fmac_f32_dpp v167, v193, v84 row_ror:14 row_mask:0xf bank_mask:0xf
+	v_fmac_f32_dpp v147, v193, v77 row_ror:7 row_mask:0xf bank_mask:0xf
+	v_fmac_f32_dpp v167, v193, v85 row_ror:15 row_mask:0xf bank_mask:0xf
+	v_add_f32_e32 v193, v147, v167
+	v_add_f32_e32 v194, v147, v167
+	s_nop 1
+	v_permlane32_swap_b32_e32 v193, v194
+	v_mul_f32_e32 v147, 0xbfb8aa3b, v193
+	v_exp_f32_e32 v147, v147
+	v_sub_f32_e32 v167, v197, v194
+	v_mul_f32_e32 v166, v167, v147
+	v_mul_f32_e32 v204, v167, v147
+	v_sub_f32_e32 v192, v192, v193
+	s_nop 0
+	v_permlane16_swap_b32_e32 v166, v204
+	s_nop 0
+	v_mov_b32_e32 v147, v166
+	v_mov_b32_e32 v193, v204
+	v_bfi_b32 v199, v173, v196, v195
+	v_mov_b32_dpp v147, v166 row_ror:8 row_mask:0xa bank_mask:0xf
+	v_mov_b32_dpp v193, v204 row_ror:8 row_mask:0xa bank_mask:0xf
+	v_fma_f32 v197, v147, v30, v26
+	v_mul_f32_e32 v198, v193, v42
+	v_fmac_f32_dpp v198, v193, v43 row_ror:1 row_mask:0xf bank_mask:0xf
+	v_fmac_f32_dpp v197, v147, v31 row_ror:1 row_mask:0xf bank_mask:0xf
+	v_fmac_f32_dpp v198, v193, v44 row_ror:2 row_mask:0xf bank_mask:0xf
+	v_fmac_f32_dpp v197, v147, v32 row_ror:2 row_mask:0xf bank_mask:0xf
+	v_fmac_f32_dpp v198, v193, v45 row_ror:3 row_mask:0xf bank_mask:0xf
+	v_fmac_f32_dpp v197, v147, v33 row_ror:3 row_mask:0xf bank_mask:0xf
+	v_fmac_f32_dpp v198, v193, v46 row_ror:4 row_mask:0xf bank_mask:0xf
+	v_fmac_f32_dpp v197, v147, v38 row_ror:4 row_mask:0xf bank_mask:0xf
+	v_fmac_f32_dpp v198, v193, v47 row_ror:5 row_mask:0xf bank_mask:0xf
+	v_fmac_f32_dpp v197, v147, v39 row_ror:5 row_mask:0xf bank_mask:0xf
+	v_fmac_f32_dpp v198, v193, v48 row_ror:6 row_mask:0xf bank_mask:0xf
+	v_fmac_f32_dpp v197, v147, v40 row_ror:6 row_mask:0xf bank_mask:0xf
+	v_fmac_f32_dpp v198, v193, v49 row_ror:7 row_mask:0xf bank_mask:0xf
+	v_fmac_f32_dpp v197, v147, v41 row_ror:7 row_mask:0xf bank_mask:0xf
+	v_add_f32_e32 v193, v197, v198
+	v_mov_b32_dpp v147, v198 row_ror:8 row_mask:0xf bank_mask:0xf
+	v_add_f32_dpp v147, v197, v147 row_ror:8 row_mask:0xf bank_mask:0xf
+	s_nop 1
+	v_permlane16_swap_b32_e32 v193, v147
+	v_add_f32_e32 v197, v193, v147
+	v_exp_f32_e32 v147, v197
+	v_max_f32_e32 v193, 0, v197
+	v_add_f32_e32 v147, 1.0, v147
+	v_rcp_f32_e32 v147, v147
+	s_nop 0
+	v_fma_f32 v147, v147, -2.0, 1.0
+	v_bfi_b32 v197, v142, v193, v147
+	v_fma_f32 v147, v197, v6, v27
+	s_nop 0
+	v_mul_f32_dpp v193, v197, v7 row_ror:1 row_mask:0xf bank_mask:0xf
+	v_fmac_f32_dpp v147, v197, v8 row_ror:2 row_mask:0xf bank_mask:0xf
+	v_fmac_f32_dpp v193, v197, v9 row_ror:3 row_mask:0xf bank_mask:0xf
+	v_fmac_f32_dpp v147, v197, v14 row_ror:4 row_mask:0xf bank_mask:0xf
+	v_fmac_f32_dpp v193, v197, v15 row_ror:5 row_mask:0xf bank_mask:0xf
+	v_fmac_f32_dpp v147, v197, v16 row_ror:6 row_mask:0xf bank_mask:0xf
+	v_fmac_f32_dpp v193, v197, v17 row_ror:7 row_mask:0xf bank_mask:0xf
+	v_add_f32_e32 v197, v147, v193
+	v_add_f32_e32 v198, v147, v193
+	s_nop 1
+	v_permlane16_swap_b32_e32 v197, v198
+	v_add_f32_e32 v197, v197, v198
+	v_exp_f32_e32 v147, v197
+	v_max_f32_e32 v193, 0, v197
+	v_add_f32_e32 v147, 1.0, v147
+	v_rcp_f32_e32 v147, v147
+	s_nop 0
+	v_fma_f32 v147, v147, -2.0, 1.0
+	v_bfi_b32 v197, v142, v193, v147
+	v_fma_f32 v147, v197, v2, v28
+	v_mov_b32_e32 v193, 0
+	v_fmac_f32_dpp v193, v197, v18 row_ror:8 row_mask:0xf bank_mask:0xf
+	v_fmac_f32_dpp v147, v197, v3 row_ror:1 row_mask:0xf bank_mask:0xf
+	v_fmac_f32_dpp v193, v197, v19 row_ror:9 row_mask:0xf bank_mask:0xf
+	v_fmac_f32_dpp v147, v197, v4 row_ror:2 row_mask:0xf bank_mask:0xf
+	v_fmac_f32_dpp v193, v197, v20 row_ror:10 row_mask:0xf bank_mask:0xf
+	v_fmac_f32_dpp v147, v197, v5 row_ror:3 row_mask:0xf bank_mask:0xf
+	v_fmac_f32_dpp v193, v197, v21 row_ror:11 row_mask:0xf bank_mask:0xf
+	v_fmac_f32_dpp v147, v197, v10 row_ror:4 row_mask:0xf bank_mask:0xf
+	v_fmac_f32_dpp v193, v197, v22 row_ror:12 row_mask:0xf bank_mask:0xf
+	v_fmac_f32_dpp v147, v197, v11 row_ror:5 row_mask:0xf bank_mask:0xf
+	v_fmac_f32_dpp v193, v197, v23 row_ror:13 row_mask:0xf bank_mask:0xf
+	v_fmac_f32_dpp v147, v197, v12 row_ror:6 row_mask:0xf bank_mask:0xf
+	v_fmac_f32_dpp v193, v197, v24 row_ror:14 row_mask:0xf bank_mask:0xf
+	v_fmac_f32_dpp v147, v197, v13 row_ror:7 row_mask:0xf bank_mask:0xf
+	v_fmac_f32_dpp v193, v197, v25 row_ror:15 row_mask:0xf bank_mask:0xf
+	v_add_f32_e32 v197, v147, v193
+	v_add_f32_e32 v198, v147, v193
+	s_nop 1
+	v_permlane32_swap_b32_e32 v197, v198
+	v_mul_f32_e32 v147, 0xbfb8aa3b, v197
+	v_exp_f32_e32 v147, v147
+	v_sub_f32_e32 v193, v199, v198
+	v_mul_f32_e32 v167, v193, v147
+	v_mul_f32_e32 v194, v193, v147
+	v_sub_f32_e32 v192, v192, v197
+	s_nop 0
+	v_permlane16_swap_b32_e32 v167, v194
+	v_mov_b32_e32 v195, v166
+	v_pk_mul_f32 v[196:197], s[52:53], v[166:167]
+	v_pk_mul_f32 v[198:199], s[52:53], v[194:195]
+	v_pk_mul_f32 v[202:203], v[196:197], v[196:197] neg_lo:[0,1] neg_hi:[0,1]
+	v_mov_b32_dpp v201, v197 row_ror:15 row_mask:0xf bank_mask:0xf bound_ctrl:1
+	v_pk_add_f32 v[202:203], v[198:199], v[202:203]
+	v_pk_add_f32 v[196:197], v[196:197], 1.0 op_sel_hi:[1,0] neg_lo:[1,0] neg_hi:[1,0]
+	v_pk_mul_f32 v[202:203], v[202:203], v[202:203]
+	v_pk_mul_f32 v[196:197], v[196:197], v[196:197]
+	v_pk_mul_f32 v[202:203], v[202:203], s[18:19] op_sel_hi:[1,0]
+	s_nop 0
+	v_pk_add_f32 v[196:197], v[196:197], v[202:203]
+	s_nop 0
+	v_cndmask_b32_e64 v147, 0, v197, s[2:3]
+	v_cndmask_b32_e64 v193, 0, v196, s[4:5]
+	v_pk_mul_f32 v[196:197], v[198:199], v[198:199]
+	v_add_f32_e32 v193, v193, v147
+	v_mul_f32_e32 v147, s52, v204
+	v_mov_b32_e32 v199, v196
+	v_pk_add_f32 v[196:197], v[146:147], v[198:199] neg_lo:[0,1] neg_hi:[0,1]
+	s_nop 0
+	v_pk_mul_f32 v[196:197], v[196:197], v[196:197]
+	s_nop 0
+	v_mul_f32_e32 v195, 0x42c80000, v197
+	v_add_f32_e32 v195, v196, v195
+	v_mul_f32_e32 v197, v147, v147
+	v_mov_b32_e32 v196, v147
+	v_pk_add_f32 v[196:197], v[200:201], v[196:197] neg_lo:[0,1] neg_hi:[0,1]
+	v_cndmask_b32_e64 v195, 0, v195, s[6:7]
+	v_pk_mul_f32 v[196:197], v[196:197], v[196:197]
+	v_add_f32_e32 v193, v195, v193
+	v_mul_f32_e32 v147, 0x42c80000, v197
+	v_add_f32_e32 v147, v196, v147
+	v_cndmask_b32_e64 v147, 0, v147, s[8:9]
+	v_add_f32_e32 v147, v147, v193
+	s_nop 1
+	v_add_f32_dpp v192, v192, v192 row_ror:8 row_mask:0xf bank_mask:0xf bound_ctrl:1
+	v_add_f32_dpp v147, v147, v147 row_ror:8 row_mask:0xf bank_mask:0xf bound_ctrl:1
+	s_nop 0
+	v_add_f32_dpp v192, v192, v192 row_ror:4 row_mask:0xf bank_mask:0xf bound_ctrl:1
+	v_add_f32_dpp v147, v147, v147 row_ror:4 row_mask:0xf bank_mask:0xf bound_ctrl:1
+	s_nop 0
+	v_add_f32_dpp v192, v192, v192 row_ror:2 row_mask:0xf bank_mask:0xf bound_ctrl:1
+	v_add_f32_dpp v147, v147, v147 row_ror:2 row_mask:0xf bank_mask:0xf bound_ctrl:1
+	s_nop 0
+	v_add_f32_dpp v193, v192, v192 row_ror:1 row_mask:0xf bank_mask:0xf bound_ctrl:1
+	v_add_f32_dpp v192, v192, v192 row_ror:1 row_mask:0xf bank_mask:0xf bound_ctrl:1
+	v_add_f32_dpp v147, v147, v147 row_ror:1 row_mask:0xf bank_mask:0xf bound_ctrl:1
+	s_nop 0
+	v_permlane16_swap_b32_e32 v192, v193
+	v_add_f32_e32 v192, v192, v193
+	s_nop 0
+	v_cvt_f64_f32_e32 v[196:197], v147
+	v_max3_f32 v147, |v204|, |v166|, |v194|
+	v_max_f32_e64 v166, |v167|, |v167|
+	v_max_f32_e32 v147, v147, v166
+	v_cmp_nlt_f32_e32 vcc, 1.0, v147
+	s_cmp_eq_u64 vcc, -1
+	v_sub_f32_e32 v147, v192, v177
+	s_cselect_b64 s[12:13], -1, 0
+	v_cndmask_b32_e64 v193, v182, v147, s[12:13]
+	v_mul_f32_e32 v166, 0x3fb8aa3b, v193
+	v_exp_f32_e32 v194, v166
+	v_cmp_le_f64_e64 vcc, |v[196:197]|, s[54:55]
+	v_min_f32_e32 v194, 1.0, v194
+	s_nop 0
+	v_cndmask_b32_e64 v167, v180, -v197, vcc
+	v_cndmask_b32_e32 v166, v181, v196, vcc
+	v_cmp_u_f32_e32 vcc, v193, v193
+	v_cmp_lt_f64_e64 s[14:15], s[26:27], v[166:167]
+	s_nop 0
+	v_cndmask_b32_e32 v193, v194, v193, vcc
+	v_cmp_lt_f32_e32 vcc, v185, v193
+	s_and_b64 s[68:69], s[50:51], vcc
+	s_and_b64 vcc, exec, s[10:11]
+	s_and_b64 s[14:15], s[68:69], s[14:15]
+	s_cbranch_vccnz 62
+	v_cvt_f64_f32_e32 v[194:195], v147
+	v_add_f64 v[196:197], v[166:167], -v[144:145]
+	v_add_f64 v[194:195], v[196:197], v[194:195]
+	v_cndmask_b32_e64 v195, v183, v195, s[12:13]
+	v_cndmask_b32_e64 v194, 0, v194, s[12:13]
+	v_mul_f64 v[196:197], v[194:195], s[56:57]
+	v_rndne_f64_e32 v[196:197], v[196:197]
+	v_fma_f64 v[198:199], s[58:59], v[196:197], v[194:195]
+	v_fmac_f64_e32 v[198:199], s[60:61], v[196:197]
+	v_mov_b64_e32 v[200:201], v[148:149]
+	v_fmac_f64_e32 v[200:201], s[62:63], v[198:199]
+	v_mov_b64_e32 v[202:203], v[150:151]
+	v_fmac_f64_e32 v[202:203], v[198:199], v[200:201]
+	v_mov_b64_e32 v[200:201], v[152:153]
+	v_fmac_f64_e32 v[200:201], v[198:199], v[202:203]
+	v_mov_b64_e32 v[202:203], v[154:155]
+	v_fmac_f64_e32 v[202:203], v[198:199], v[200:201]
+	v_mov_b64_e32 v[200:201], v[156:157]
+	v_fmac_f64_e32 v[200:201], v[198:199], v[202:203]
+	v_mov_b64_e32 v[202:203], v[158:159]
+	v_fmac_f64_e32 v[202:203], v[198:199], v[200:201]
+	v_mov_b64_e32 v[200:201], v[160:161]
+	v_fmac_f64_e32 v[200:201], v[198:199], v[202:203]
+	v_mov_b64_e32 v[202:203], v[162:163]
+	v_fmac_f64_e32 v[202:203], v[198:199], v[200:201]
+	v_mov_b64_e32 v[200:201], v[164:165]
+	v_fmac_f64_e32 v[200:201], v[198:199], v[202:203]
+	v_fma_f64 v[200:201], v[198:199], v[200:201], 1.0
+	v_fma_f64 v[198:199], v[198:199], v[200:201], 1.0
+	v_cvt_i32_f64_e32 v147, v[196:197]
+	v_ldexp_f64 v[196:197], v[198:199], v147
+	v_min_f64 v[196:197], v[196:197], 1.0
+	v_cmp_nlt_f64_e32 vcc, s[64:65], v[194:195]
+	v_cmp_ngt_f64_e64 s[12:13], s[66:67], v[194:195]
+	s_andn2_b64 s[14:15], s[14:15], exec
+	v_cndmask_b32_e32 v147, v184, v197, vcc
+	s_and_b64 vcc, s[12:13], vcc
+	v_cndmask_b32_e64 v195, 0, v147, s[12:13]
+	v_cndmask_b32_e32 v194, 0, v196, vcc
+	v_cvt_f64_f32_e32 v[196:197], v185
+	v_cmp_gt_f64_e32 vcc, v[194:195], v[196:197]
+	s_and_b64 s[12:13], s[50:51], vcc
+	s_and_b64 s[12:13], s[12:13], exec
+	s_or_b64 s[14:15], s[14:15], s[12:13]
+	v_mov_b32_e32 v147, v175
+	v_cndmask_b32_e64 v185, 0, 1, s[14:15]
+	s_and_saveexec_b64 s[12:13], s[16:17]
+	s_cbranch_execz 64298
+	s_branch 64294
```

New measurement: 1.010 billion, median of 6. 7.3% higher.
